# guohaoqiang/Flex

Hardware: AMD Instinct MI355X
Metric: SpMM GFLOPS (2*nnz*k/t) (higher is better)
Workload: dtype f32

## Files before the change

flex_amd/binding.py:

```python
from __future__ import annotations

import ctypes as C
import os
import subprocess

import numpy as np

_HERE = os.path.dirname(os.path.abspath(__file__))
_CSRC = os.path.join(_HERE, "csrc")
_SO = os.path.join(_HERE, "lib", "libflex_spmm.so")

FLEX_ORDER_NATURAL = 0
FLEX_ORDER_RCM = 1
FLEX_ORDER_CLUSTER = 2
FLEX_ORDER_GORDER = 3
FLEX_PLAN_STATS = 0x100
FLEX_PLAN_AUTOTUNE = 0x200
FLEX_PLAN_ROW_RANGE = 0x1000
FLEX_PLAN_XCD_INTERLEAVE = 0x2000
FLEX_PLAN_TRANSPOSE = 0x8000
FLEX_PLAN_MUTABLE_VALUES = 0x10000
FLEX_PLAN_ATTENTION = 0x40000
FLEX_PLAN_ATTENTION_BACKWARD = 0x80000
FLEX_PLAN_BF16 = 0x100000


class FlexError(RuntimeError):
    pass


class _Csr(C.Structure):
    _fields_ = [("m", C.c_int32), ("n", C.c_int32), ("nnz", C.c_int64),
                ("rowPtr", C.c_void_p), ("col", C.c_void_p), ("vals", C.c_void_p)]


class _HostCsr(C.Structure):
    _fields_ = [("m", C.c_int32), ("n", C.c_int32), ("nnz", C.c_int64),
                ("rowPtr", C.POINTER(C.c_uint32)), ("col", C.POINTER(C.c_uint32)),
                ("vals", C.POINTER(C.c_float)),
                ("uni_nb", C.c_int64), ("n_edges_one_way", C.c_int64),
                ("n_edges_asymmetric", C.c_int64),
                ("n_nodes_z_out", C.c_int32), ("n_nodes_z_in", C.c_int32),
                ("n_nodes_z_deg", C.c_int32), ("is_directed", C.c_int32), ("c", C.c_int32)]


class _PlanInfo(C.Structure):
    _fields_ = [("m", C.c_int32), ("n", C.c_int32), ("k", C.c_int32), ("device", C.c_int32),
                ("nnz", C.c_int64), ("n_tasks", C.c_int64), ("n_chunks", C.c_int64),
                ("n_split_rows", C.c_int64), ("n_partials", C.c_int64),
                ("device_bytes", C.c_int64), ("lanes_per_nz", C.c_int32), ("order", C.c_int32),
                ("plan_ms", C.c_double), ("n_slots", C.c_int64), ("two_d", C.c_int32), ("panel_rows", C.c_int32),
                ("n_tiles", C.c_int64), ("tile_nnz", C.c_int64), ("n_records", C.c_int64),
                ("n_blocks", C.c_int64), ("block_rows", C.c_int64), ("block_nnz", C.c_int64), ("block_hot_nnz", C.c_int64),
                ("block_hot_cols", C.c_int64), ("block_panels", C.c_int64), ("block_records", C.c_int64),
                ("n_bundles", C.c_int64), ("bundle_rows", C.c_int64)]


class _PlanStats(C.Structure):
    _fields_ = [("records", C.c_int64), ("cols_wave", C.c_int64), ("cols_wg", C.c_int64),
                ("cols_xcd", C.c_int64), ("reuse_wave", C.c_double), ("reuse_wg", C.c_double),
                ("reuse_xcd", C.c_double), ("gather_bytes", C.c_double), ("l2_bytes", C.c_double),
                ("chunk_rec_max", C.c_int64), ("chunk_rec_mean", C.c_double),
                ("chunk_imb_pct", C.c_double), ("xcd_imb_pct", C.c_double),
                ("split_nnz_pct", C.c_double), ("pad_pct", C.c_double), ("n_workgroups", C.c_int64),
                ("tile_nnz_pct_10", C.c_double), ("tile_nnz_pct_25", C.c_double), ("tile_nnz_pct_50", C.c_double),
                ("tile_mean_fill", C.c_double), ("mfma_tiles", C.c_int64), ("mfma_nnz_pct", C.c_double),
                ("lds_hot_pct_2", C.c_double), ("lds_hot_pct_4", C.c_double), ("lds_u_2", C.c_double), ("lds_u_4", C.c_double)]


class _ClusterTuning(C.Structure):
    _fields_ = [(f, C.c_int32) for f in ("batch", "no_refine", "stretch", "sweeps", "stride")]


class _PlanTuning(C.Structure):
    _fields_ = [(f, C.c_int32) for f in (
        "lanes_per_nz", "chunk_records", "long_row", "piece_records", "row_cost", "xcd_slices", "xcd_balance",
        "chunk_cost", "task_cost", "split_rows", "rec_nt", "unroll", "two_d", "panel_kb", "seg_min", "mfma",
        "mfma_fill_pct", "lds_extra", "host_threads")] + [("cluster", _ClusterTuning)] + [(f, C.c_int32) for f in (
        "blocks", "block_rounds", "block_panel_rows", "block_thr", "block_cap", "block_ablate_retired", "tile_group", "xcd_stretch", "far_first", "bundle", "bundle_len", "rec_pack")] + [("reserved", C.c_int32 * 4)]


TUNING_FIELDS = tuple(f for f, _ in _PlanTuning._fields_ if f not in ("cluster", "block_ablate_retired", "reserved"))
CLUSTER_TUNING_FIELDS = tuple(f for f, _ in _ClusterTuning._fields_)


DEFAULT_TUNING: dict = {}


def _tuning(d) -> "_PlanTuning | None":
    if not d:
        return None
    t = _PlanTuning()
    for key, val in d.items():
        if key in TUNING_FIELDS:
            setattr(t, key, int(val))
        elif key.startswith("cluster_") and key[8:] in CLUSTER_TUNING_FIELDS:
            setattr(t.cluster, key[8:], int(val))
        else:
            raise FlexError(f"unknown tuning knob {key!r} (flex_plan_tuning has: {', '.join(TUNING_FIELDS)}, cluster_*)")
    return t


class _PlanDesc(C.Structure):
    _fields_ = [("struct_size", C.c_size_t), ("A", C.POINTER(_Csr)), ("k", C.c_int), ("ldb", C.c_int), ("ldc", C.c_int),
                ("device", C.c_int), ("flags", C.c_uint), ("row_begin", C.c_int64), ("row_end", C.c_int64),
                ("col_map", C.c_void_p), ("row_map", C.c_void_p), ("tuning", C.POINTER(_PlanTuning))]


class _KernelInfo(C.Structure):
    _fields_ = [("vgprs", C.c_int32), ("sgprs", C.c_int32), ("lds_bytes", C.c_int32), ("scratch_bytes", C.c_int32),
                ("threads_per_block", C.c_int32), ("waves_per_cu", C.c_int32)]


class _Imbalance(C.Structure):
    _fields_ = [("waves", C.c_int64), ("cus_seen", C.c_int32), ("xcds_seen", C.c_int32), ("span_us", C.c_double),
                ("cu_busy_imb_pct", C.c_double), ("cu_end_spread_pct", C.c_double), ("xcd_busy_imb_pct", C.c_double),
                ("xcd_end_spread_pct", C.c_double), ("wave_us_mean", C.c_double), ("wave_us_max", C.c_double)]


class _SoftmaxInfo(C.Structure):
    _fields_ = [(f, C.c_int64) for f in ("rows", "entries", "items", "groups", "rows_empty", "rows_packed", "rows_wave", "rows_block",
                                          "group_entries", "device_bytes")]


class _AttentionInfo(C.Structure):
    _fields_ = [(f, C.c_int64) for f in ("rows", "entries", "items", "groups", "rows_empty", "rows_slot", "rows_wave", "rows_block",
                                          "group_budget", "device_bytes")]


class _AttentionBackwardInfo(C.Structure):
    _fields_ = [(f, C.c_int64) for f in ("columns", "entries", "items", "groups", "columns_empty", "columns_slot", "columns_wave", "columns_block",
                                          "group_budget", "device_bytes")]


class _RecordInfo(C.Structure):
    _fields_ = [("packed", C.c_int32), ("reserved", C.c_int32)] + [(f, C.c_int64) for f in ("records", "wide_records", "exceptions", "stream_bytes")]


class _SynthParams(C.Structure):
    _fields_ = [("n", C.c_int64), ("nnz", C.c_int64), ("alpha", C.c_double),
                ("community", C.c_int64), ("p_in", C.c_double), ("p_near", C.c_double),
                ("near_window", C.c_int32), ("shuffle", C.c_int32), ("gcn_norm", C.c_int32),
                ("directed", C.c_int32), ("seed", C.c_uint64)]


SYMBOLS = [
    "flex_plan_create", "flex_plan_create_ex", "flex_plan_create_ld", "flex_plan_create_mapped", "flex_plan_create_rows", "flex_spmm",
    "flex_plan_destroy", "flex_plan_measure_imbalance", "flex_plan_get_info", "flex_plan_get_stats", "flex_plan_get_tuning", "flex_set_host_threads", "flex_order_cluster_ex", "flex_plan_self_check", "flex_plan_kernel_info", "flex_hbm_probe", "flex_gather_rows", "flex_csv_load", "flex_mtx_load",
    "flex_csv_save", "flex_csr_save_bin", "flex_csr_load_bin", "flex_csr_fingerprint", "flex_perm_save", "flex_perm_load",
    "flex_host_csr_free", "flex_fill_dense_rand", "flex_order_rcm", "flex_order_cluster", "flex_order_gorder", "flex_perm_csr",
    "flex_order_deg", "flex_order_dfs", "flex_order_rabbit", "flex_shard_rows", "flex_synth_graph", "flex_synth_preset", "flex_strerror", "flex_last_hip_error",
    "flex_last_hip_error_string", "flex_abi_version", "flex_plan_set_values", "flex_sddmm",
    "flex_edge_softmax", "flex_edge_softmax_backward", "flex_plan_softmax_info", "flex_attention", "flex_plan_attention_info",
    "flex_attention_backward", "flex_plan_attention_backward_info", "flex_attention_heads", "flex_attention_heads_backward",
    "flex_gat_attention", "flex_gat_attention_backward", "flex_plan_record_info", "flex_plan_read_records",
    "flex_attention_bf16", "flex_attention_bf16_backward", "flex_spmm_bf16", "flex_plan_is_bf16",
    "flex_attention_bias", "flex_attention_bias_backward", "flex_attention_bf16_bias", "flex_attention_bf16_bias_backward",
    "flex_attention_dropout", "flex_attention_dropout_backward", "flex_attention_bf16_dropout", "flex_attention_bf16_dropout_backward",
    "flex_dropout_mask", "flex_gat_attention_dropout", "flex_gat_attention_dropout_backward",
]

_lib = None


def lib_path() -> str:
    return _SO


def build(force: bool = False) -> str:
    if force and os.path.exists(_SO):
        os.remove(_SO)
    subprocess.check_call(["make", "-s", "-C", _CSRC, "all"])
    return _SO


def lib():
    global _lib
    if _lib is None:
        if not os.path.exists(_SO):
            raise FlexError(f"{_SO} is missing: run `python -c 'import __graft_entry__ as g; g.build()'` "
                            "(there is no CPU fallback)")
        try:
            import torch
        except ImportError:
            pass
        L = C.CDLL(_SO)
        vp, i64, i32, u32 = C.c_void_p, C.c_int64, C.c_int, C.c_uint
        L.flex_plan_create.argtypes = [C.POINTER(vp), C.POINTER(_Csr), i32, i32, u32]
        L.flex_plan_create_ex.argtypes = [C.POINTER(vp), C.POINTER(_PlanDesc)]
        L.flex_plan_create_ld.argtypes = [C.POINTER(vp), C.POINTER(_Csr), i32, i32, i32, i32, u32]
        L.flex_plan_create_mapped.argtypes = [C.POINTER(vp), C.POINTER(_Csr), vp, i32, i32, u32]
        L.flex_plan_create_rows.argtypes = [C.POINTER(vp), C.POINTER(_Csr), i64, i64, vp, i32, i32, u32]
        L.flex_spmm.argtypes = [vp, vp, vp, vp]
        L.flex_plan_destroy.argtypes = [vp]
        L.flex_plan_get_info.argtypes = [vp, C.POINTER(_PlanInfo)]
        L.flex_plan_get_stats.argtypes = [vp, C.POINTER(_PlanStats)]
        L.flex_plan_get_tuning.argtypes = [vp, C.POINTER(_PlanTuning)]
        L.flex_set_host_threads.argtypes = [i32]
        L.flex_order_cluster_ex.argtypes = [C.POINTER(_Csr), C.POINTER(_ClusterTuning), vp]
        L.flex_plan_self_check.argtypes = [vp]
        L.flex_plan_measure_imbalance.argtypes = [vp, vp, vp, vp, C.POINTER(_Imbalance)]
        L.flex_plan_kernel_info.argtypes = [vp, C.POINTER(_KernelInfo)]
        L.flex_gather_rows.argtypes = [vp, vp, vp, i64, i32, vp]
        L.flex_hbm_probe.argtypes = [i32, i64, i32, i32, C.POINTER(C.c_double), C.POINTER(C.c_double)]
        L.flex_csv_load.argtypes = [C.c_char_p, C.POINTER(_HostCsr)]
        L.flex_mtx_load.argtypes = [C.c_char_p, i32, C.POINTER(_HostCsr)]
        L.flex_csv_save.argtypes = [C.c_char_p, C.POINTER(_Csr)]
        L.flex_csr_fingerprint.argtypes = [C.POINTER(_Csr)]
        L.flex_csr_fingerprint.restype = C.c_uint64
        L.flex_perm_save.argtypes = [C.c_char_p, vp, i64, C.c_uint64]
        L.flex_perm_load.argtypes = [C.c_char_p, vp, i64, C.c_uint64]
        L.flex_csr_save_bin.argtypes = [C.c_char_p, C.POINTER(_Csr)]
        L.flex_csr_load_bin.argtypes = [C.c_char_p, C.POINTER(_HostCsr)]
        L.flex_host_csr_free.argtypes = [C.POINTER(_HostCsr)]
        L.flex_host_csr_free.restype = None
        L.flex_fill_dense_rand.argtypes = [vp, i64, i32]
        L.flex_order_rcm.argtypes = [C.POINTER(_Csr), vp]
        L.flex_order_cluster.argtypes = [C.POINTER(_Csr), vp]
        L.flex_order_gorder.argtypes = [C.POINTER(_Csr), u32, vp]
        L.flex_order_dfs.argtypes = [C.POINTER(_Csr), vp]
        L.flex_order_rabbit.argtypes = [C.POINTER(_Csr), i32, vp]
        L.flex_order_deg.argtypes = [C.POINTER(_Csr), i32, vp]
        L.flex_synth_preset.argtypes = [C.c_char_p, i32, C.POINTER(_SynthParams)]
        L.flex_perm_csr.argtypes = [C.POINTER(_Csr), vp, vp, vp, vp, vp]
        L.flex_shard_rows.argtypes = [C.POINTER(_Csr), i32, i32, vp]
        L.flex_synth_graph.argtypes = [C.POINTER(_SynthParams), C.POINTER(_HostCsr)]
        L.flex_strerror.argtypes = [i32]
        L.flex_strerror.restype = C.c_char_p
        L.flex_last_hip_error.restype = i32
        L.flex_last_hip_error_string.restype = C.c_char_p
        L.flex_abi_version.restype = i32
        L.flex_plan_softmax_info.argtypes = [vp, C.POINTER(_SoftmaxInfo)]
        L.flex_plan_attention_info.argtypes = [vp, C.POINTER(_AttentionInfo)]
        L.flex_plan_attention_backward_info.argtypes = [vp, C.POINTER(_AttentionBackwardInfo)]
        L.flex_plan_record_info.argtypes = [vp, C.POINTER(_RecordInfo)]
        L.flex_plan_read_records.argtypes = [vp, vp, i64]
        L.flex_plan_is_bf16.argtypes = [vp]
        L.flex_dropout_mask.argtypes = [C.c_uint64, C.c_float, C.c_uint64, C.c_uint64, vp]
        _lib = L
    return _lib


def _values_fn(name: str):
    L = lib()
    f = getattr(L, name)
    if f.argtypes is None:
        vp, fl, i32, u64 = C.c_void_p, C.c_float, C.c_int, C.c_uint64
        f.argtypes = {"flex_plan_set_values": [vp, vp, vp], "flex_sddmm": [vp, vp, vp, vp, vp], "flex_edge_softmax": [vp, vp, fl, vp, vp],
                      "flex_edge_softmax_backward": [vp, vp, vp, fl, vp, vp], "flex_attention": [vp, vp, vp, vp, fl, vp, vp, vp],
                      "flex_attention_backward": [vp, vp, vp, vp, vp, vp, fl, vp, vp, vp, vp, vp],
                      "flex_attention_heads": [vp, i32, vp, vp, vp, fl, vp, vp, vp],
                      "flex_attention_heads_backward": [vp, i32, vp, vp, vp, vp, vp, fl, vp, vp, vp, vp, vp],
                      "flex_attention_bf16": [vp, i32, vp, vp, vp, fl, vp, vp, vp],
                      "flex_attention_bf16_backward": [vp, i32, vp, vp, vp, vp, vp, fl, vp, vp, vp, vp, vp],
                      "flex_attention_bias": [vp, i32, vp, vp, vp, vp, fl, vp, vp, vp],
                      "flex_attention_bias_backward": [vp, i32, vp, vp, vp, vp, vp, fl, vp, vp, vp, vp, vp, vp],
                      "flex_attention_bf16_bias": [vp, i32, vp, vp, vp, vp, fl, vp, vp, vp],
                      "flex_attention_bf16_bias_backward": [vp, i32, vp, vp, vp, vp, vp, fl, vp, vp, vp, vp, vp, vp],
                      "flex_attention_dropout": [vp, i32, vp, vp, vp, vp, fl, fl, u64, vp, vp, vp],
                      "flex_attention_dropout_backward": [vp, i32, vp, vp, vp, vp, vp, fl, fl, u64, vp, vp, vp, vp, vp, vp],
                      "flex_attention_bf16_dropout": [vp, i32, vp, vp, vp, vp, fl, fl, u64, vp, vp, vp],
                      "flex_attention_bf16_dropout_backward": [vp, i32, vp, vp, vp, vp, vp, fl, fl, u64, vp, vp, vp, vp, vp, vp],
                      "flex_spmm_bf16": [vp, vp, vp, vp],
                      "flex_gat_attention": [vp, i32, vp, vp, vp, fl, vp, vp, vp],
                      "flex_gat_attention_backward": [vp, i32, vp, vp, vp, vp, vp, fl, vp, vp, vp, vp, vp],
                      "flex_gat_attention_dropout": [vp, i32, vp, vp, vp, fl, fl, u64, vp, vp, vp],
                      "flex_gat_attention_dropout_backward": [vp, i32, vp, vp, vp, vp, vp, fl, fl, u64, vp, vp, vp, vp, vp]}[name]
    return f


def _check(rc: int, what: str):
    if rc != 0:
        L = lib()
        msg = L.flex_strerror(rc).decode()
        if rc == -3:
            msg += f" [hip {L.flex_last_hip_error()}: {L.flex_last_hip_error_string().decode()}]"
        raise FlexError(f"{what}: {msg} ({rc})")


class HostCsr:

    def __init__(self, rowPtr, col, vals, n=None, **stats):
        self.rowPtr = np.ascontiguousarray(rowPtr, dtype=np.uint32)
        self.col = np.ascontiguousarray(col, dtype=np.uint32)
        self.vals = np.ascontiguousarray(vals, dtype=np.float32)
        self.m = len(self.rowPtr) - 1
        self.n = self.m if n is None else int(n)
        self.nnz = len(self.col)
        self.__dict__.update(stats)

    def view(self) -> _Csr:
        return _Csr(self.m, self.n, self.nnz, self.rowPtr.ctypes.data, self.col.ctypes.data,
                    self.vals.ctypes.data)


def _take(s: _HostCsr) -> HostCsr:
    n = s.n
    try:
        rp = np.ctypeslib.as_array(s.rowPtr, shape=(s.m + 1,)).copy()
        col = np.ctypeslib.as_array(s.col, shape=(max(s.nnz, 1),))[: s.nnz].copy()
        vals = np.ctypeslib.as_array(s.vals, shape=(max(s.nnz, 1),))[: s.nnz].copy()
        stats = {k: getattr(s, k) for k in ("uni_nb", "n_edges_one_way", "n_edges_asymmetric",
                                           "n_nodes_z_out", "n_nodes_z_in", "n_nodes_z_deg",
                                           "is_directed", "c")}
    finally:
        lib().flex_host_csr_free(C.byref(s))
    return HostCsr(rp, col, vals, n=n, **stats)


def csv_load(path: str) -> HostCsr:
    s = _HostCsr()
    _check(lib().flex_csv_load(os.fsencode(path), C.byref(s)), f"flex_csv_load({path})")
    return _take(s)


def mtx_load(path: str, sort_columns: bool = True) -> HostCsr:
    s = _HostCsr()
    _check(lib().flex_mtx_load(os.fsencode(path), int(sort_columns), C.byref(s)), f"flex_mtx_load({path})")
    return _take(s)
# ... 110 lines not shown
def order_gorder(a: HostCsr, window: int = 3) -> np.ndarray:
    rank = np.empty(max(a.m, 1), dtype=np.uint32)
    v = a.view()
    _check(lib().flex_order_gorder(C.byref(v), int(window), rank.ctypes.data), "flex_order_gorder")
    return rank[: a.m]


def order_dfs(a: HostCsr) -> np.ndarray:
    rank = np.empty(max(a.m, 1), dtype=np.uint32)
    v = a.view()
    _check(lib().flex_order_dfs(C.byref(v), rank.ctypes.data), "flex_order_dfs")
    return rank[: a.m]


def order_rabbit(a: HostCsr, is_directed: bool | None = None) -> np.ndarray:
    if is_directed is None:
        is_directed = bool(getattr(a, "is_directed", 0))
    rank = np.empty(max(a.m, 1), dtype=np.uint32)
    v = a.view()
    _check(lib().flex_order_rabbit(C.byref(v), int(bool(is_directed)), rank.ctypes.data), "flex_order_rabbit")
    return rank[: a.m]


def order_deg(a: HostCsr, descending: bool = True) -> np.ndarray:
    rank = np.empty(max(a.m, 1), dtype=np.uint32)
    v = a.view()
    _check(lib().flex_order_deg(C.byref(v), int(descending), rank.ctypes.data), "flex_order_deg")
    return rank[: a.m]


class Plan:

    def __init__(self, a: HostCsr, k: int, device: int = 0, order: int = FLEX_ORDER_NATURAL,
                 vo_mp=None, rows=None, col_map=None, ldb: int | None = None, ldc: int | None = None, tuning: dict | None = None,
                 transpose: bool = False, mutable_values: bool = False, attention: bool = False, attention_backward: bool = False,
                 bf16: bool = False):
        self._h = C.c_void_p()
        self.src_nnz = a.nnz
        if transpose:
            order |= FLEX_PLAN_TRANSPOSE
        if mutable_values:
            order |= FLEX_PLAN_MUTABLE_VALUES
        if attention:
            order |= FLEX_PLAN_ATTENTION
        if attention_backward:
            order |= FLEX_PLAN_ATTENTION_BACKWARD
        if bf16:
            order |= FLEX_PLAN_BF16
        self._keep = (a, vo_mp, col_map)
        v = a.view()
        L = lib()
        tn = _tuning({**DEFAULT_TUNING, **(tuning or {})})
        if tn is not None or ((ldb is not None or ldc is not None) and (rows is not None or vo_mp is not None)):
            cm = None if col_map is None else np.ascontiguousarray(col_map, dtype=np.int32)
            vm = None if vo_mp is None else np.ascontiguousarray(vo_mp, dtype=np.int32)
            self._keep = (a, cm, vm)
            d = _PlanDesc(C.sizeof(_PlanDesc), C.pointer(v), k, ldb or 0, ldc or 0, device,
                          order | (0 if rows is None else FLEX_PLAN_ROW_RANGE),
                          0 if rows is None else int(rows[0]), 0 if rows is None else int(rows[1]),
                          (cm if cm is not None else vm).ctypes.data if (cm is not None or vm is not None) else None,
                          None if vm is None else vm.ctypes.data, None if tn is None else C.pointer(tn))
            rc = L.flex_plan_create_ex(C.byref(self._h), C.byref(d))
        elif rows is not None:
            cm = None if col_map is None else np.ascontiguousarray(col_map, dtype=np.int32)
            self._keep = (a, cm)
            rc = L.flex_plan_create_rows(C.byref(self._h), C.byref(v), int(rows[0]), int(rows[1]),
                                         None if cm is None else cm.ctypes.data, k, device, order)
        elif vo_mp is not None:
            vm = np.ascontiguousarray(vo_mp, dtype=np.int32)
            rc = L.flex_plan_create_mapped(C.byref(self._h), C.byref(v), vm.ctypes.data, k, device, order)
        elif ldb is not None or ldc is not None:
            rc = L.flex_plan_create_ld(C.byref(self._h), C.byref(v), k, ldb or k, ldc or k, device, order)
        else:
            rc = L.flex_plan_create(C.byref(self._h), C.byref(v), k, device, order)
        _check(rc, "flex_plan_create")
        self.k = k
        self._keep = None

    def info(self) -> dict:
        i = _PlanInfo()
        _check(lib().flex_plan_get_info(self._h, C.byref(i)), "flex_plan_get_info")
        d = {f: getattr(i, f) for f, _ in _PlanInfo._fields_}
        d["rec_packed"] = self.record_info()["packed"]
        d["bf16"] = int(lib().flex_plan_is_bf16(self._h))
        return d

    def record_info(self) -> dict:
        ri = _RecordInfo()
        _check(lib().flex_plan_record_info(self._h, C.byref(ri)), "flex_plan_record_info")
        return {f: getattr(ri, f) for f, _ in _RecordInfo._fields_ if f != "reserved"}

    def records(self) -> np.ndarray:
        n = self.record_info()["records"]
        out = np.empty((max(n, 1), 2), dtype=np.uint32)
        _check(lib().flex_plan_read_records(self._h, out.ctypes.data, n), "flex_plan_read_records")
        return out[:n]

    def stats(self) -> dict:
        st = _PlanStats()
        _check(lib().flex_plan_get_stats(self._h, C.byref(st)), "flex_plan_get_stats")
        return {f: getattr(st, f) for f, _ in _PlanStats._fields_}

    def tuning(self) -> dict:
        t = _PlanTuning()
        _check(lib().flex_plan_get_tuning(self._h, C.byref(t)), "flex_plan_get_tuning")
        d = {f: getattr(t, f) for f in TUNING_FIELDS}
        d.update({"cluster_" + f: getattr(t.cluster, f) for f in CLUSTER_TUNING_FIELDS})
        return d

    def kernel_info(self) -> dict:
        ki = _KernelInfo()
        _check(lib().flex_plan_kernel_info(self._h, C.byref(ki)), "flex_plan_kernel_info")
        return {f: getattr(ki, f) for f, _ in _KernelInfo._fields_}

    def measure_imbalance(self, dB_ptr: int, dC_ptr: int, stream: int = 0) -> dict:
        im = _Imbalance()
        _check(lib().flex_plan_measure_imbalance(self._h, dB_ptr, dC_ptr, stream, C.byref(im)), "flex_plan_measure_imbalance")
        return {f: getattr(im, f) for f, _ in _Imbalance._fields_}

    def self_check(self):
        _check(lib().flex_plan_self_check(self._h), "flex_plan_self_check")

    def spmm(self, dB_ptr: int, dC_ptr: int, stream: int = 0):
        _check(lib().flex_spmm(self._h, dB_ptr, dC_ptr, stream), "flex_spmm")

    def spmm_bf16(self, dB_ptr: int, dC_ptr: int, stream: int = 0):
        _check(_values_fn("flex_spmm_bf16")(self._h, dB_ptr, dC_ptr, stream), "flex_spmm_bf16")

    def __call__(self, B, out=None):
        import torch
        i = self.info()
        want = torch.bfloat16 if i["bf16"] else torch.float32
        if B.dtype != want:
            raise TypeError(f"this plan takes {want} operands, got {B.dtype}")
        assert B.is_cuda and B.is_contiguous() and tuple(B.shape) == (i["n"], i["k"])
        if out is None:
            out = torch.empty((i["m"], i["k"]), dtype=want, device=B.device)
        elif out.dtype != want:
            raise TypeError(f"this plan writes {want}, out is {out.dtype}")
        run = self.spmm_bf16 if i["bf16"] else self.spmm
        run(B.data_ptr(), out.data_ptr(), torch.cuda.current_stream(B.device).cuda_stream)
        return out

    def set_values(self, vals, stream: int | None = None):
        import torch
        assert vals.is_cuda and vals.dtype == torch.float32 and vals.is_contiguous() and vals.numel() == self.src_nnz, "float32 cuda [nnz]"
        s = torch.cuda.current_stream(vals.device).cuda_stream if stream is None else stream
        _check(_values_fn("flex_plan_set_values")(self._h, vals.data_ptr(), s), "flex_plan_set_values")

    def sddmm_ptr(self, dG_ptr: int, dB_ptr: int, dOut_ptr: int, stream: int = 0):
        _check(_values_fn("flex_sddmm")(self._h, dG_ptr, dB_ptr, dOut_ptr, stream), "flex_sddmm")

    def sddmm(self, G, B, out=None):
        import torch
        i = self.info()
        assert G.is_cuda and G.dtype == torch.float32 and G.is_contiguous() and tuple(G.shape) == (i["m"], i["k"])
        assert B.is_cuda and B.dtype == torch.float32 and B.is_contiguous() and tuple(B.shape) == (i["n"], i["k"])
        if out is None:
            out = torch.zeros(self.src_nnz, dtype=torch.float32, device=G.device)
        assert out.is_cuda and out.dtype == torch.float32 and out.is_contiguous() and out.numel() == self.src_nnz
        self.sddmm_ptr(G.data_ptr(), B.data_ptr(), out.data_ptr(), torch.cuda.current_stream(G.device).cuda_stream)
        return out

    def softmax_info(self) -> dict:
        i = _SoftmaxInfo()
        _check(lib().flex_plan_softmax_info(self._h, C.byref(i)), "flex_plan_softmax_info")
        return {f: getattr(i, f) for f, _ in _SoftmaxInfo._fields_}

    def edge_softmax_ptr(self, dScores_ptr: int, scale: float, dOut_ptr: int, stream: int = 0):
        _check(_values_fn("flex_edge_softmax")(self._h, dScores_ptr, scale, dOut_ptr, stream), "flex_edge_softmax")

    def edge_softmax_backward_ptr(self, dP_ptr: int, dGradP_ptr: int, scale: float, dGradS_ptr: int, stream: int = 0):
        _check(_values_fn("flex_edge_softmax_backward")(self._h, dP_ptr, dGradP_ptr, scale, dGradS_ptr, stream), "flex_edge_softmax_backward")

    def _edge_vectors(self, *ts):
        import torch
        for t in ts:
            assert t.is_cuda and t.dtype == torch.float32 and t.is_contiguous() and t.numel() == self.src_nnz, "float32 cuda [nnz]"
# ... 403 lines not shown
```

flex_amd/csrc/plan.cpp:

```cpp
#include <algorithm>
#include <atomic>
#include <chrono>
#include <cstddef>
#include <cstdlib>
#include <memory>
#include <new>
#include <vector>

#include "host_parallel.h"
#include "plan.h"

namespace flex {

static thread_local hipError_t g_last_hip = hipSuccess;
void note_hip_error(hipError_t e) { g_last_hip = e; }

int validate_csr(const flex_csr *A) {
    if (!A || A->m < 0 || A->n < 0 || A->nnz < 0) return FLEX_ERR_INVALID;
    if (!A->rowPtr) return FLEX_ERR_INVALID;
    if (A->nnz > 0 && (!A->col || !A->vals)) return FLEX_ERR_INVALID;
    if (A->nnz >= (int64_t(1) << 32)) return FLEX_ERR_UNSUPPORTED;
    if (A->rowPtr[0] != 0 || A->rowPtr[A->m] != static_cast<uint32_t>(A->nnz)) return FLEX_ERR_INVALID;
    for (int32_t r = 0; r < A->m; ++r)
        if (A->rowPtr[r] > A->rowPtr[r + 1]) return FLEX_ERR_INVALID;
// ... 97 lines not shown
    flex_csr csr{};
};

static int transpose_csr(const flex_csr *A, TransposedCsr *t, bool want_entries) {
    int rc = validate_csr(A);
    if (rc) return rc;
    if (A->n >= INT32_MAX) return FLEX_ERR_UNSUPPORTED;
    const size_t nnz = static_cast<size_t>(A->nnz);
    try {
        t->rowPtr.assign(static_cast<size_t>(A->n) + 1, 0u);
        t->col.resize(nnz);
        t->vals.resize(nnz);
        if (want_entries) t->entry.resize(nnz);
    } catch (const std::bad_alloc &) {
        return FLEX_ERR_NOMEM;
    }
    for (size_t e = 0; e < nnz; ++e) ++t->rowPtr[A->col[e] + 1];
    for (int32_t c = 0; c < A->n; ++c) t->rowPtr[c + 1] += t->rowPtr[c];
    std::vector<uint32_t> pos;
    try {
        pos.assign(t->rowPtr.begin(), t->rowPtr.end() - 1);
    } catch (const std::bad_alloc &) {
        return FLEX_ERR_NOMEM;
    }
    for (int32_t r = 0; r < A->m; ++r)
        for (uint32_t e = A->rowPtr[r]; e < A->rowPtr[r + 1]; ++e) {
            const uint32_t d = pos[A->col[e]]++;
            t->col[d] = static_cast<uint32_t>(r);
            t->vals[d] = A->vals[e];
            if (want_entries) t->entry[d] = e;
        }
    t->csr = flex_csr{A->n, A->m, A->nnz, t->rowPtr.data(), nnz ? t->col.data() : nullptr, nnz ? t->vals.data() : nullptr};
    return FLEX_OK;
}

static uint64_t held_entries_fp(const flex_csr *A, bool transposed, int64_t r0, int64_t r1, const int32_t *col_map) {
    auto brow = [&](uint32_t c) { return col_map ? static_cast<uint32_t>(col_map[c]) : c; };
    uint64_t fp = 0;
    if (!transposed) {
        for (uint32_t e = A->rowPtr[r0]; e < A->rowPtr[r1]; ++e) fp += entry_fp(e, brow(A->col[e]));
        return fp;
    }
    for (int32_t r = 0; r < A->m; ++r)
        for (uint32_t e = A->rowPtr[r]; e < A->rowPtr[r + 1]; ++e)
            if (A->col[e] >= r0 && A->col[e] < r1) fp += entry_fp(e, brow(static_cast<uint32_t>(r)));
    return fp;
}

static int create_common(flex_plan **out, const flex_csr *hostA, bool all_rows, int64_t row_begin, int64_t row_end,
                         const int32_t *col_map, const int32_t *dst_map, int k, int device, unsigned flags,
                         int ldb = 0, int ldc = 0, const flex_plan_tuning *tuning_in = nullptr) {
    if (!out) return FLEX_ERR_INVALID;
    *out = nullptr;
    flex_plan_tuning tuning = tuning_in ? *tuning_in : flex_plan_tuning{};
    if (!tuning_ok(tuning)) return FLEX_ERR_INVALID;
    const HostThreadsScope threads_for_this_call(tuning.host_threads);
    if (k <= 0 || device < 0) return FLEX_ERR_INVALID;
    if (ldb == 0) ldb = k;
    if (ldc == 0) ldc = k;
    if (ldb < k || ldc < k) return FLEX_ERR_INVALID;
    const unsigned order = flags & FLEX_ORDER_MASK;
    if (order > FLEX_ORDER_GORDER ||
        (flags & ~(FLEX_ORDER_MASK | FLEX_PLAN_STATS | FLEX_PLAN_AUTOTUNE | FLEX_PLAN_XCD_INTERLEAVE | FLEX_PLAN_TRANSPOSE | FLEX_PLAN_MUTABLE_VALUES | FLEX_PLAN_ATTENTION | FLEX_PLAN_ATTENTION_BACKWARD | FLEX_PLAN_BF16)))
        return FLEX_ERR_INVALID;
    const bool bf16 = (flags & FLEX_PLAN_BF16) != 0;
    if (bf16) {
        if (flags & (FLEX_PLAN_MUTABLE_VALUES | FLEX_PLAN_ATTENTION | FLEX_PLAN_ATTENTION_BACKWARD | FLEX_PLAN_AUTOTUNE)) return FLEX_ERR_UNSUPPORTED;
        if (k % 8 != 0 || ldb % 8 != 0 || ldc % 8 != 0) return FLEX_ERR_UNSUPPORTED;
        if (tuning.mfma == 1 || tuning.blocks == 1 || tuning.split_rows == 1 || tuning.two_d == 1) return FLEX_ERR_UNSUPPORTED;
        tuning.mfma = 2;
        tuning.blocks = 2;
        tuning.split_rows = 2;
        k /= 2;
        ldb /= 2;
        ldc /= 2;
        flags &= ~FLEX_PLAN_BF16;
    }
    const bool mut = (flags & FLEX_PLAN_MUTABLE_VALUES) != 0;
    if (mut) {
        if (tuning.mfma == 1 || tuning.blocks == 1 || tuning.rec_pack == 1) return FLEX_ERR_UNSUPPORTED;
        tuning.mfma = 2;
        tuning.blocks = 2;
        tuning.rec_pack = 2;
    }
    int rc = FLEX_OK;
    const flex_csr *const callerA = hostA;
    const bool transposed = (flags & FLEX_PLAN_TRANSPOSE) != 0;
    const bool attn = (flags & FLEX_PLAN_ATTENTION) != 0;
    if (attn && (transposed || col_map || dst_map || tuning.rec_pack == 1)) return FLEX_ERR_UNSUPPORTED;
    if (attn) tuning.rec_pack = 2;
    const bool attn_bwd = (flags & FLEX_PLAN_ATTENTION_BACKWARD) != 0;
    if (attn_bwd && !attn) return FLEX_ERR_INVALID;
    if (attn_bwd && !all_rows) return FLEX_ERR_UNSUPPORTED;
    flags &= ~(FLEX_PLAN_ATTENTION | FLEX_PLAN_ATTENTION_BACKWARD);
    TransposedCsr at;
    if (transposed) {
        rc = transpose_csr(hostA, &at, mut);
        if (rc) return rc;
        hostA = &at.csr;
        flags &= ~FLEX_PLAN_TRANSPOSE;
    }
    rc = validate_csr(hostA);
    if (rc) return rc;
    if (hostA->m >= INT32_MAX) return FLEX_ERR_UNSUPPORTED;
    if (all_rows) {
        row_begin = 0;
        row_end = hostA->m;
    }
    if (row_begin < 0 || row_end < row_begin || row_end > hostA->m) return FLEX_ERR_INVALID;
    if (col_map)
        for (int32_t c = 0; c < hostA->n; ++c)
            if (col_map[c] < 0 || col_map[c] >= hostA->n) return FLEX_ERR_INVALID;
    if (dst_map)
        for (int64_t r = row_begin; r < row_end; ++r)
            if (dst_map[r] < 0 || dst_map[r] >= hostA->m) return FLEX_ERR_INVALID;
    const auto t0 = std::chrono::steady_clock::now();
    const DeviceScope on(device);
    FLEX_HIP_TRY(on.error());
    std::unique_ptr<flex_plan> p(new (std::nothrow) flex_plan());
    if (!p) return FLEX_ERR_NOMEM;
    p->m = static_cast<int32_t>(row_end - row_begin);
    p->n = hostA->n;
    p->k = k;
    p->ldb = ldb;
    p->ldc = ldc;
    p->bf16 = bf16;
    p->nnz = static_cast<int64_t>(hostA->rowPtr[row_end]) - hostA->rowPtr[row_begin];
    p->device = device;
    std::vector<uint32_t> sched_cache;
    const bool tune = (flags & FLEX_PLAN_AUTOTUNE) != 0;
    const uint32_t *entry_of = transposed && mut && hostA->nnz > 0 ? at.entry.data() : nullptr;
    try {
        rc = build_plan(p.get(), hostA, static_cast<int32_t>(row_begin), static_cast<int32_t>(row_end), col_map, dst_map, flags, tuning,
                        tune ? &sched_cache : nullptr, 0, entry_of);
        if (rc == FLEX_OK && tune) rc = autotune(p, hostA, static_cast<int32_t>(row_begin), static_cast<int32_t>(row_end), col_map, dst_map, flags, tuning, sched_cache, entry_of);
        if (rc == FLEX_OK && mut) {
            p->src_nnz = callerA->nnz;
            p->ent_fp = held_entries_fp(callerA, transposed, row_begin, row_end, col_map);
            if (!transposed) rc = upload_softmax_image(p.get(), callerA->rowPtr, row_begin, row_end);
            else if (all_rows) rc = upload_softmax_image(p.get(), callerA->rowPtr, 0, callerA->m);
        }
        if (rc == FLEX_OK && attn) {
            p->at_ent_fp = held_entries_fp(callerA, false, row_begin, row_end, nullptr);
            if (attn_bwd)
                for (int32_t r = 0; r < callerA->m; ++r)
                    for (uint32_t e = callerA->rowPtr[r]; e < callerA->rowPtr[r + 1]; ++e) p->ab_fp += rowptr_fp(static_cast<uint32_t>(r), e);
            rc = upload_attention_image(p.get(), callerA, row_begin, row_end, attn_bwd);
        }
    } catch (const std::bad_alloc &) {
        rc = FLEX_ERR_NOMEM;
    } catch (...) {
        rc = FLEX_ERR_INVALID;
    }
    if (rc == FLEX_OK && hipDeviceSynchronize() != hipSuccess) rc = FLEX_ERR_HIP;
    if (rc) return rc;
    p->plan_ms = std::chrono::duration<double, std::milli>(std::chrono::steady_clock::now() - t0).count();
    *out = p.release();
    return FLEX_OK;
}

int flex_plan_create(flex_plan **out, const flex_csr *hostA, int k, int device, unsigned flags) {
    if (!hostA) return FLEX_ERR_INVALID;
    return create_common(out, hostA, true, 0, 0, nullptr, nullptr, k, device, flags);
}

int flex_plan_create_ld(flex_plan **out, const flex_csr *hostA, int k, int ldb, int ldc, int device, unsigned flags) {
    if (!hostA || ldb < k || ldc < k) return FLEX_ERR_INVALID;
    return create_common(out, hostA, true, 0, 0, nullptr, nullptr, k, device, flags, ldb, ldc);
}

int flex_plan_create_mapped(flex_plan **out, const flex_csr *hostA, const int32_t *vo_mp, int k, int device,
                            unsigned flags) {
    if (!hostA) return FLEX_ERR_INVALID;
    if (vo_mp && hostA->m != hostA->n) return FLEX_ERR_INVALID;
    return create_common(out, hostA, true, 0, 0, vo_mp, vo_mp, k, device, flags);
}

int flex_plan_create_rows(flex_plan **out, const flex_csr *hostA, int64_t row_begin, int64_t row_end,
                          const int32_t *col_map, int k, int device, unsigned flags) {
    if ((flags & FLEX_ORDER_MASK) != FLEX_ORDER_NATURAL) return FLEX_ERR_INVALID;
    return create_common(out, hostA, false, row_begin, row_end, col_map, nullptr, k, device, flags);
}

int flex_plan_create_ex(flex_plan **out, const flex_plan_desc *d) {
    constexpr size_t kSizeAbi2 = offsetof(flex_plan_desc, tuning);
    if (!d || !d->A || (d->struct_size != sizeof(flex_plan_desc) && d->struct_size != kSizeAbi2)) return FLEX_ERR_INVALID;
    const flex_plan_tuning *tuning = d->struct_size == sizeof(flex_plan_desc) ? d->tuning : nullptr;
    const bool all_rows = (d->flags & FLEX_PLAN_ROW_RANGE) == 0;
    if (all_rows && (d->row_begin != 0 || d->row_end != 0)) return FLEX_ERR_INVALID;
    const int64_t r0 = d->row_begin, r1 = d->row_end;
    if (d->row_map && (!all_rows || d->A->m != d->A->n)) return FLEX_ERR_INVALID;
    if (!all_rows && (d->flags & FLEX_ORDER_MASK) != FLEX_ORDER_NATURAL) return FLEX_ERR_INVALID;
    return create_common(out, d->A, all_rows, r0, r1, d->col_map, d->row_map, d->k, d->device, d->flags & ~FLEX_PLAN_ROW_RANGE, d->ldb, d->ldc, tuning);
}

int flex_spmm(flex_plan *p, const float *dB, float *dC, flex_stream_t stream) {
    if (!p || p->bf16) return FLEX_ERR_INVALID;
    if (p->m == 0) return FLEX_OK;
    if (!dC || (!dB && p->nnz > 0)) return FLEX_ERR_INVALID;
    const DeviceScope on(p->device);
    FLEX_HIP_TRY(on.error());
    const bool vec4 = operands_vec4(p, dB, dC);
    const bool fused = vec4 && p->fused_fixup;
    hipStream_t s = reinterpret_cast<hipStream_t>(stream);
    int rc = FLEX_OK;
    const LaunchGuard guard(p, s);
    if (guard.begin() != FLEX_OK) return FLEX_ERR_INVALID;
    rc = launch_spmm(plan_view(p, fused, nullptr), p->lanes_per_nz, p->off32, vec4, dB, dC, s, p->unroll);
    if (rc == FLEX_OK && !fused) rc = launch_fixup(p->d_partial.get(), p->d_split.get(), p->n_split, p->k, p->ldc, dC, s);
    if (rc == FLEX_OK && p->n_tiles) rc = launch_tiles(tile_view(p), p->off32, dB, dC, p->k, p->ldb, p->ldc, s);
    if (rc == FLEX_OK && p->bk_blocks) rc = launch_blocks(block_view(p), dB, dC, s, vec4);
    if (rc == FLEX_OK) guard.done();
    return rc;
}

int flex_plan_destroy(flex_plan *p) {
    if (!p) return FLEX_OK;
    const DeviceScope on(p->device);
    delete p;
    return FLEX_OK;
}

int flex_plan_get_info(const flex_plan *p, flex_plan_info *o) {
    if (!p || !o) return FLEX_ERR_INVALID;
    o->m = p->m;
    o->n = p->n;
    o->k = p->k * p->elems_per_word();
    o->device = p->device;
    o->nnz = p->nnz;
    o->n_tasks = p->n_tasks;
    o->n_chunks = p->n_chunks;
    o->n_split_rows = p->n_split;
    o->n_partials = p->n_partials;
    o->device_bytes = p->device_bytes;
    o->lanes_per_nz = p->lanes_per_nz;
    o->order = static_cast<int32_t>(p->order);
    o->plan_ms = p->plan_ms;
    o->n_slots = p->n_slots;
    o->two_d = p->two_d ? 1 : 0;
    o->n_tiles = p->n_tiles;
    o->tile_nnz = p->tile_nnz;
    o->n_records = p->n_records;
    o->panel_rows = p->two_d ? static_cast<int32_t>(p->panel_rows) : 0;
    o->n_blocks = p->bk_blocks;
    o->block_rows = p->bk_rows;
    o->block_nnz = p->bk_nnz;
    o->block_hot_nnz = p->bk_hot_nnz;
    o->block_hot_cols = p->bk_hot_cols;
    o->block_panels = p->bk_panels;
    o->block_records = static_cast<int64_t>(p->d_bk_rec.size());
    o->n_bundles = p->n_bundles;
    o->bundle_rows = p->bundle_rows;
    return FLEX_OK;
}

int flex_plan_record_info(const flex_plan *p, flex_record_info *o) {
    if (!p || !o) return FLEX_ERR_INVALID;
    const int64_t exceptions = static_cast<int64_t>(p->d_exc.size());
    const int64_t bytes = p->rec_packed ? 6 * (p->n_records - p->wide_records) + 8 * (p->wide_records + exceptions) : 8 * p->n_records;
    *o = flex_record_info{p->rec_packed ? 1 : 0, 0, p->n_records, p->wide_records, exceptions, bytes};
    return FLEX_OK;
}

int flex_plan_softmax_info(const flex_plan *p, flex_softmax_info *o) {
    if (!p || !o || !p->mutable_vals) return FLEX_ERR_INVALID;
    if (!p->sm_ok) return FLEX_ERR_UNSUPPORTED;
    *o = flex_softmax_info{p->sm_rows, p->sm_entries, static_cast<int64_t>(p->d_sm_item.size()), p->n_sm_groups, p->sm_class_rows[3],
                           p->sm_class_rows[kSmPacked], p->sm_class_rows[kSmWaveRow], p->sm_class_rows[kSmBlockRow], p->sm_group_budget, p->sm_bytes};
    return FLEX_OK;
}

int flex_plan_attention_backward_info(const flex_plan *p, flex_attention_backward_info *o) {
    if (!p || !o || !p->ab_ok) return FLEX_ERR_INVALID;
    *o = flex_attention_backward_info{p->ab_cols, p->at_entries, static_cast<int64_t>(p->d_ab_item.size()), p->n_ab_groups, p->ab_class_cols[3],
                                      p->ab_class_cols[kAtSlot], p->ab_class_cols[kAtWave], p->ab_class_cols[kAtBlock], p->ab_group_budget, p->ab_bytes};
    return FLEX_OK;
}

int flex_plan_attention_info(const flex_plan *p, flex_attention_info *o) {
    if (!p || !o || !p->at_ok) return FLEX_ERR_INVALID;
    *o = flex_attention_info{p->at_rows, p->at_entries, static_cast<int64_t>(p->d_at_item.size()), p->n_at_groups, p->at_class_rows[3],
                             p->at_class_rows[kAtSlot], p->at_class_rows[kAtWave], p->at_class_rows[kAtBlock], p->at_group_budget, p->at_bytes};
    return FLEX_OK;
}

// ... 68 lines not shown
```

flex_amd/csrc/plan.h:

```cpp
#pragma once
#include <algorithm>
#include <cstdlib>
#include <memory>
#include <new>
#include <type_traits>
#include <utility>
#include <vector>

#include "internal.h"

namespace flex {

template <class T>
class DeviceArray {
  public:
    DeviceArray() = default;
    DeviceArray(DeviceArray &&o) noexcept : ptr_(std::exchange(o.ptr_, nullptr)), n_(std::exchange(o.n_, 0)) {}
    DeviceArray &operator=(DeviceArray o) noexcept {
        std::swap(ptr_, o.ptr_);
        std::swap(n_, o.n_);
        return *this;
    }
    ~DeviceArray() { if (ptr_) (void)hipFree(ptr_); }
    T *get() const { return ptr_; }
    size_t size() const { return n_; }
    hipError_t allocate(size_t n) {
        *this = DeviceArray();
        const hipError_t e = hipMalloc(reinterpret_cast<void **>(&ptr_), std::max<size_t>(n, 1) * sizeof(T));
        if (e != hipSuccess) ptr_ = nullptr;
        else n_ = n;
        return e;
    }
    template <class A>
    int upload(const std::vector<T, A> &h, int64_t *device_bytes) {
        FLEX_HIP_TRY(allocate(h.size()));
        if (!h.empty()) FLEX_HIP_TRY(hipMemcpy(ptr_, h.data(), h.size() * sizeof(T), hipMemcpyHostToDevice));
        *device_bytes += static_cast<int64_t>(std::max<size_t>(h.size(), 1) * sizeof(T));
        return FLEX_OK;
    }

  private:
    T *ptr_ = nullptr;
    size_t n_ = 0;
};

class DeviceScope {
  public:
    explicit DeviceScope(int dev) {
        err_ = hipGetDevice(&prev_);
        if (err_ == hipSuccess && prev_ != dev) {
            err_ = hipSetDevice(dev);
            switched_ = err_ == hipSuccess;
        }
    }
    ~DeviceScope() { if (switched_) (void)hipSetDevice(prev_); }
    DeviceScope(const DeviceScope &) = delete;
    DeviceScope &operator=(const DeviceScope &) = delete;
    hipError_t error() const { return err_; }

  private:
    int prev_ = -1;
    bool switched_ = false;
    hipError_t err_ = hipSuccess;
};

}

struct flex_plan {
    int32_t m = 0, n = 0, k = 0, device = 0;
    int32_t ldb = 0, ldc = 0;
    bool bf16 = false;
    int elems_per_word() const { return bf16 ? 2 : 1; }
    int64_t nnz = 0;
    int lanes_per_nz = 0;
    bool off32 = false;
    bool xcd_remap = true;
    unsigned lds_extra = 0;
    bool rec_nt = false;
    uint32_t tile_group = 0;
    int unroll = 0;
    unsigned order = 0;
    flex::DeviceArray<uint2> d_rec;
    flex::DeviceArray<uint32_t> d_t_beg, d_t_dst;
    flex::DeviceArray<uint2> d_t_aux;
    flex::DeviceArray<uint4> d_chunk;
    flex::DeviceArray<uint32_t> d_bd_rows;
    flex::DeviceArray<uint2> d_chunk_bd;
    bool rec_packed = false;
    flex::DeviceArray<float> d_rec_val;
    flex::DeviceArray<uint16_t> d_rec_dcol;
    flex::DeviceArray<uint32_t> d_t_col0;
    flex::DeviceArray<uint2> d_chunk_exc, d_exc;
    int64_t n_records = 0;
    int64_t wide_records = 0;
    uint64_t rec_fp = 0;
    uint32_t n_bundles = 0;
    int64_t bundle_rows = 0;
    flex::DeviceArray<float> d_partial;
    flex::DeviceArray<flex::SplitRow> d_split;
    flex::DeviceArray<uint32_t> d_split_cnt;
    bool fused_fixup = false;
    bool two_d = false;
    flex::DeviceArray<float> d_tile_a;
    flex::DeviceArray<uint32_t> d_tile_boff, d_tile_mask, d_rt_ptr, d_rt_rows;
    uint32_t n_tiles = 0, n_row_tiles = 0;
    int64_t tile_nnz = 0;
    int64_t tile_hist[3] = {0, 0, 0}, tile_cells = 0;
    bool tile_hist_valid = false;
    uint32_t panel_rows = 0;
    flex::DeviceArray<uint4> d_bk_hdr;
    flex::DeviceArray<uint2> d_bk_wstart, d_bk_rec;
    flex::DeviceArray<uint32_t> d_bk_cnt, d_bk_hcol, d_bk_brow, d_bk_link;
    uint32_t bk_blocks = 0, bk_rounds = 0, bk_panel_rows = 0;
    int64_t bk_rows = 0, bk_nnz = 0, bk_hot_nnz = 0, bk_hot_cols = 0, bk_panels = 0;
    uint32_t n_tasks = 0, n_chunks = 0, n_slots = 0, n_split = 0, n_partials = 0;
    int64_t c_rows = 0;
    int64_t device_bytes = 0;
    double plan_ms = 0;
    double lds_hot[2] = {0, 0}, lds_u[2] = {0, 0};
    bool has_stats = false;
    flex_plan_stats stats{};
    flex_plan_tuning tuning{};
    hipStream_t last_stream = nullptr;
    bool launched = false;
    bool mutable_vals = false;
    flex::DeviceArray<uint32_t> d_src;
    flex::DeviceArray<float> d_vrec;
    flex::DeviceArray<uint4> d_seg;
    flex::DeviceArray<uint4> d_sd_item;
    flex::DeviceArray<uint32_t> d_sd_grp;
    uint32_t n_sd_groups = 0;
    int64_t src_nnz = 0;
    uint64_t ent_fp = 0;
    bool sm_ok = false;
    flex::DeviceArray<uint32_t> d_sm_rowptr;
    flex::DeviceArray<uint4> d_sm_item;
    flex::DeviceArray<uint32_t> d_sm_grp;
    uint32_t n_sm_groups = 0, n_sm_wave_items = 0, n_sm_block_rows = 0, sm_group_budget = 0;
    int64_t sm_rows = 0, sm_entries = 0, sm_bytes = 0;
    int64_t sm_class_rows[4] = {0, 0, 0, 0};
    uint64_t sm_fp = 0;
    bool at_ok = false;
    flex::DeviceArray<uint32_t> d_at_rowptr;
    flex::DeviceArray<uint32_t> d_at_src;
    flex::DeviceArray<uint4> d_at_item;
    flex::DeviceArray<uint32_t> d_at_grp;
    uint32_t n_at_groups = 0, n_at_wave_items = 0, n_at_block_rows = 0, at_group_budget = 0, at_first_entry = 0;
    int64_t at_rows = 0, at_entries = 0, at_bytes = 0;
    int64_t at_class_rows[4] = {0, 0, 0, 0};
    uint64_t at_fp = 0, at_ent_fp = 0;
    bool ab_ok = false;
    flex::DeviceArray<uint32_t> d_ab_colptr;
    flex::DeviceArray<uint2> d_ab_ent;
    flex::DeviceArray<uint4> d_ab_item;
    flex::DeviceArray<uint32_t> d_ab_grp;
    uint32_t n_ab_groups = 0, n_ab_wave_items = 0, n_ab_block_cols = 0, ab_group_budget = 0;
    int64_t ab_cols = 0, ab_bytes = 0;
    int64_t ab_class_cols[4] = {0, 0, 0, 0};
    uint64_t ab_fp = 0;
};

namespace flex {


template <typename T>
struct default_init_allocator : std::allocator<T> {
    template <typename U>
    struct rebind {
        using other = default_init_allocator<U>;
    };
    template <typename U>
    void construct(U *ptr) noexcept(std::is_nothrow_default_constructible_v<U>) {
        ::new (static_cast<void *>(ptr)) U;
    }
    template <typename U, typename... Args>
    void construct(U *ptr, Args &&...args) {
        ::new (static_cast<void *>(ptr)) U(std::forward<Args>(args)...);
    }
};
using RecordVec = std::vector<uint2, default_init_allocator<uint2>>;

inline PlanView plan_view(const flex_plan *p, bool fused, uint64_t *trace) {
    return PlanView{p->d_rec.get(), p->d_t_beg.get(), p->d_t_dst.get(), p->d_t_aux.get(), p->d_chunk.get(), p->d_partial.get(), p->d_split.get(),
                    p->d_split_cnt.get(), fused ? 1u : 0u, p->n_slots, p->k, p->ldb, p->ldc,
                    p->xcd_remap ? 1u : 0u, p->lds_extra, p->rec_nt ? 1u : 0u, p->tile_group, trace, p->d_bd_rows.get(), p->d_chunk_bd.get(),
// ... 99 lines not shown
```

flex_amd/csrc/plan_build.cpp:

```cpp
#include <algorithm>
#include <atomic>
#include <chrono>
#include <cstdio>
#include <cmath>
#include <cstring>
#include <new>
#include <numeric>

#include "host_parallel.h"
#include "plan.h"

namespace flex {

namespace {

struct Piece {
    uint32_t spos;
    uint32_t beg, end;
    uint32_t phase;
    uint32_t own_chunk;
};
constexpr uint32_t kFarPhase = 0xFFFFFFFEu;
struct TaskSpec {
    uint32_t ref;
    uint32_t rows;
    uint32_t steps;
};
constexpr uint32_t kMaxTasksPerWave = 63;

class PlanBuilder {
   public:
    PlanBuilder(flex_plan *plan, const flex_csr *csr, int32_t row_begin, int32_t row_end, const int32_t *col_map_, const int32_t *dst_map_,
                unsigned flags_, const flex_plan_tuning &tuning, std::vector<uint32_t> *sched_cache_, int force_G_, bool want_blocks_ = false,
                const uint32_t *entry_of_ = nullptr)
        : p(plan), A(csr), r0(row_begin), r1(row_end), m(row_end - row_begin), k(plan->k), col_map(col_map_), dst_map(dst_map_),
          flags(flags_), order(flags_ & FLEX_ORDER_MASK), force_G(force_G_), want_blocks(want_blocks_), mut((flags_ & FLEX_PLAN_MUTABLE_VALUES) != 0),
          entry_of(entry_of_), tn(tuning), sched(sched_cache_ ? *sched_cache_ : sched_local),
          have_cache(sched_cache_ != nullptr), timing(plan_timing_enabled()), t_last(std::chrono::steady_clock::now()) {}

    int schedule_only(std::vector<uint32_t> **sched_out, std::vector<uint32_t> **colpos_out) {
        if (order > FLEX_ORDER_GORDER) return FLEX_ERR_INVALID;
        if (order != FLEX_ORDER_NATURAL && (A->m != A->n || r0 != 0 || r1 != A->m)) return FLEX_ERR_INVALID;
        choose_tile_width();
        const int rc = order_rows();
        lap("row schedule");
        *sched_out = &sched;
        *colpos_out = &colpos;
        return rc;
    }

    int run() {
        if (order > FLEX_ORDER_GORDER) return FLEX_ERR_INVALID;
        if (order != FLEX_ORDER_NATURAL && (A->m != A->n || r0 != 0 || r1 != A->m)) return FLEX_ERR_INVALID;
        p->order = order;
        int rc;
        choose_tile_width();
        if ((rc = order_rows())) return rc;
        lap("row schedule");
        if ((flags & FLEX_PLAN_STATS) && m > 0) {
            p->lds_hot[0] = 100.0 * estimate_hot_share(A, sched, 480, 2, 4, &p->lds_u[0]);
            p->lds_hot[1] = 100.0 * estimate_hot_share(A, sched, 480, 4, 4, &p->lds_u[1]);
        }
        if ((rc = route_dense_tiles())) return rc;
        lap("dense-tile detector");
        if (want_blocks && tiles.nnz == 0 && m > 0) {
            if ((rc = route_hot_blocks())) return rc;
            lap("hot blocks");
        }
        if (mut && (tiles.nnz || p->bk_blocks)) return FLEX_ERR_UNSUPPORTED;
        read_knobs();
        if ((rc = cut_rows_into_pieces())) return rc;
        lap("pieces");
        slice_rows_for_xcds();
        order_pieces();
        lap("emission order");
        number_split_rows();
        form_tasks();
        if ((rc = pack_tasks_into_chunks())) return rc;
        fill_records();
        lap("records and tasks");
        pack_records();
        lap("record packing");
        if ((rc = upload_tasks())) return rc;
        lap("upload records/tasks");
        if ((rc = build_chunk_table())) return rc;
        lap("chunk table, stats");
        if (mut) {
            if ((rc = upload_value_image())) return rc;
            lap("value image");
        }
        return FLEX_OK;
    }

   private:
    flex_plan *const p;
    const flex_csr *A;
    const int32_t r0, r1, m;
    const int k;
    const int32_t *const col_map;
    const int32_t *const dst_map;
    const unsigned flags, order;
    const int force_G;
    const bool want_blocks;
    const bool mut;
    const uint32_t *const entry_of;
    const flex_plan_tuning &tn;
    std::vector<uint32_t> sched_local;
    std::vector<uint32_t> &sched;
    const bool have_cache;
    const bool timing;
    std::chrono::steady_clock::time_point t_last;

    int G = 8;
    uint32_t S = 8;
    double avg_deg = 0.0;
    std::vector<uint32_t> colpos;
    DenseTiles tiles;
    flex_csr A_f{};
    std::vector<uint32_t> f_rowptr, f_col;
    std::vector<float> f_vals;
    uint32_t wave_nnz = 0, row_cost = 16, long_row = 0, piece_len = 0, seg_min = 4, pshift = 0, far_window = 0;
    bool two_d = false;
    bool xcd_dealt = false;
    std::vector<Piece> pieces;
    std::vector<uint32_t> row_first_piece;
    std::vector<uint32_t> pcol;
    std::vector<float> pval;
    std::vector<uint32_t> pent;
    const uint32_t *rcol = nullptr;
    const float *rval = nullptr;
    uint32_t slice_row[kXcds + 1] = {0};
    std::vector<uint32_t> emit;
    bool bundles_on = false;
    uint32_t bundle_len = 0;
    std::vector<TaskSpec> tasks;
    std::vector<uint32_t> bundle_piece;
    std::vector<uint32_t> bd_rows;
    std::vector<uint2> chunk_bd;
    uint32_t n_bundles = 0;
    int64_t bundle_rows = 0;
    std::vector<SplitRow> split;
    std::vector<uint32_t> row_sidx, row_first_partial;
    uint32_t n_partials = 0;
    int64_t split_nnz = 0;
    std::vector<uint32_t> t_beg, t_dst, w_task;
    std::vector<uint2> t_aux;
    RecordVec rec;
    std::vector<uint32_t> rsrc;
    std::vector<float> rvals;
    uint32_t slice_chunk[kXcds + 1] = {0};
    size_t n_records = 0;
    int pack_mode = 0;
    bool packed = false;
    std::vector<float, default_init_allocator<float>> pk_val;
    std::vector<uint16_t, default_init_allocator<uint16_t>> pk_dcol;
    std::vector<uint32_t> pk_col0;
    std::vector<uint2> pk_exc, pk_chunk_exc;
    RecordVec pk_wide;
    int64_t pk_wide_records = 0;

    void lap(const char *what) {
        if (!timing) return;
        const auto now = std::chrono::steady_clock::now();
        std::fprintf(stderr, "plan: %-22s %8.1f ms\n", what, std::chrono::duration<double, std::milli>(now - t_last).count());
        t_last = now;
    }
    static long pick(int32_t given, long rule) { return given > 0 ? given : rule; }
    uint32_t dst_of(uint32_t r) const { return dst_map ? static_cast<uint32_t>(dst_map[r]) : r - static_cast<uint32_t>(r0); }
    int64_t slice_nnz() const { return static_cast<int64_t>(A->rowPtr[r1]) - A->rowPtr[r0]; }

    void choose_tile_width() {
        avg_deg = m > 0 ? static_cast<double>(A->rowPtr[r1] - A->rowPtr[r0]) / m : 0.0;
        G = 8;
        while (4 * G < k && G < 64) G <<= 1;
        const bool narrow_ok = k <= 16 && k % 4 == 0;
        if (force_G) {
            G = std::min(G, force_G);
        } else if (const int g_t = tn.lanes_per_nz; g_t == 8 || g_t == 16 || g_t == 32 || g_t == 64 || (g_t == 4 && narrow_ok)) {
            G = g_t == 4 ? 4 : std::min<int>(G, g_t);
        } else if (narrow_ok && (avg_deg >= 8.0 || tn.bundle == 1 || (tn.bundle != 2 && bundle_rule()))) {
            G = 4;
        } else {
            G = std::min(G, 32);
            if (avg_deg >= 24.0) G = std::min(G, 16);
            if (avg_deg >= 128.0) G = std::min(G, 8);
            if (tn.bundle == 1 || (tn.bundle != 2 && bundle_rule())) G = std::min(G, 16);
        }
        S = 64u / static_cast<uint32_t>(G);
        p->lanes_per_nz = G;
        p->off32 = static_cast<uint64_t>(A->n) * static_cast<uint64_t>(p->ldb) * 4u <= (uint64_t(1) << 32);
    }

    int order_rows() {
        if (have_cache && sched.size() == static_cast<size_t>(m) && m > 0) {
        } else if (sched.assign(static_cast<size_t>(m), 0u); order != FLEX_ORDER_NATURAL) {
            std::vector<uint32_t> rank;
            const int rc = order == FLEX_ORDER_RCM       ? order_rcm_host(m, A->rowPtr, A->col, rank)
                           : order == FLEX_ORDER_CLUSTER ? order_cluster_host(m, A->rowPtr, A->col, rank, &tn.cluster)
                                                         : order_gorder_host(m, A->rowPtr, A->col, 3, rank);
            if (rc) {
                sched.clear();
                return rc;
            }
            for (int32_t r = 0; r < m; ++r) sched[rank[r]] = static_cast<uint32_t>(r);
        } else {
// ... 70 lines not shown
    int route_hot_blocks() {
        BlockKnobs kn;
        const int32_t rd = tn.block_rounds;
        if (rd == 2 || rd == 4 || rd == 8) kn.rounds = static_cast<uint32_t>(rd);
        else if (rd != 0) return FLEX_ERR_INVALID;
        else if (m < 8 * 256 * 480) kn.rounds = m < 8 * 256 * 240 ? 2 : 4;
        if (tn.block_panel_rows) {
            if (tn.block_panel_rows % 4 != 0 || tn.block_panel_rows > static_cast<int32_t>(kBkPanelMax)) return FLEX_ERR_INVALID;
            kn.panel_rows = static_cast<uint32_t>(tn.block_panel_rows);
        }
        kn.thr = tn.block_thr ? static_cast<uint32_t>(tn.block_thr) : 3u;
        kn.cap = tn.block_cap ? static_cast<uint32_t>(std::min<int32_t>(tn.block_cap, 60000)) : static_cast<uint32_t>(std::clamp(1.5 * avg_deg, 32.0, 4096.0));
        kn.min_last_panel = std::min<uint32_t>(32, kn.panel_rows / 4);
        BlockImage img;
        std::vector<uint8_t> hot_mask;
        const uint32_t row_bytes32 = static_cast<uint32_t>(p->ldb) * 4u;
        int rc;
        if ((rc = build_blocks(A, sched, colpos, col_map, dst_map, r0, row_bytes32, kn, img, hot_mask))) return rc;
        flex_plan_tuning &u = p->tuning;
        u.blocks = 1;
        u.block_rounds = static_cast<int32_t>(kn.rounds);
        u.block_panel_rows = static_cast<int32_t>(kn.panel_rows);
        u.block_thr = static_cast<int32_t>(kn.thr);
        u.block_cap = static_cast<int32_t>(kn.cap);
        if (timing)
            std::fprintf(stderr, "plan: hot blocks %u x %u slots, %lld rows, %lld nnz; candidates %.1f %%, hot %.1f %% (left cold: panel budget %.1f %%, short last panel %.1f %%, runs beyond %u steps %.1f %%), "
                         "u %.2f, records / hot %.2f, panels / block %.1f\n", img.n_blocks, kn.rounds * kBkRowsPerRound, static_cast<long long>(img.rows), static_cast<long long>(img.nnz),
                         100.0 * img.cand_nnz / std::max<int64_t>(img.nnz, 1), 100.0 * img.hot_nnz / std::max<int64_t>(img.nnz, 1), 100.0 * img.lost_panels / std::max<int64_t>(img.nnz, 1),
                         100.0 * img.lost_last / std::max<int64_t>(img.nnz, 1), kn.run_max, 100.0 * img.lost_run / std::max<int64_t>(img.nnz, 1),
                         static_cast<double>(img.hot_nnz) / std::max<int64_t>(img.hot_cols, 1), static_cast<double>(img.rec.size()) / std::max<int64_t>(img.hot_nnz, 1),
                         static_cast<double>(img.panels) / std::max<uint32_t>(img.n_blocks, 1));
        if (img.hot_nnz == 0) return FLEX_OK;
        if ((rc = p->d_bk_hdr.upload(img.hdr, &p->device_bytes))) return rc;
        if ((rc = p->d_bk_wstart.upload(img.wstart, &p->device_bytes))) return rc;
        if ((rc = p->d_bk_cnt.upload(img.cnt, &p->device_bytes))) return rc;
        if ((rc = p->d_bk_hcol.upload(img.hcol, &p->device_bytes))) return rc;
        if ((rc = p->d_bk_brow.upload(img.brow, &p->device_bytes))) return rc;
        if ((rc = p->d_bk_link.upload(img.link, &p->device_bytes))) return rc;
        if ((rc = p->d_bk_rec.upload(img.rec, &p->device_bytes))) return rc;
        p->bk_blocks = img.n_blocks;
        p->bk_rounds = img.rounds;
        p->bk_panel_rows = img.panel_rows;
        p->bk_rows = img.rows;
        p->bk_nnz = img.nnz;
        p->bk_hot_nnz = img.hot_nnz;
        p->bk_hot_cols = img.hot_cols;
        p->bk_panels = img.panels;
        img = BlockImage{};
        keep_unmarked(hot_mask);
        choose_tile_width();
        return FLEX_OK;
    }

    void read_knobs() {
        const long lo_budget = G <= 8 ? 128 : 96;
        long auto_budget = std::clamp<long>(static_cast<long>((G <= 8 ? 16.0 : 8.0) * avg_deg), lo_budget, G <= 8 ? 512 : 256);
        const bool bundles_expected = tn.two_d != 1 && S >= kBundleMinSlots && m > 0 && (tn.bundle == 1 || (tn.bundle != 2 && bundle_rule()));
        const long n_rec = static_cast<long>(A->rowPtr[r1] - A->rowPtr[r0]);
        auto_budget = std::min(auto_budget, std::max<long>(G <= 8 || bundles_expected ? 64 : lo_budget, n_rec / 2048));
        wave_nnz = static_cast<uint32_t>(pick(tn.chunk_records, auto_budget));
        row_cost = static_cast<uint32_t>(pick(tn.row_cost, 16));
        const long remap_env = tn.xcd_slices;
        const bool interleave = order == FLEX_ORDER_RCM || order == FLEX_ORDER_GORDER || (flags & FLEX_PLAN_XCD_INTERLEAVE) != 0;
        p->xcd_remap = remap_env == 1 || remap_env == 3 || (remap_env != 2 && !interleave);
        xcd_dealt = remap_env == 3;
        p->lds_extra = static_cast<unsigned>(std::max(0, tn.lds_extra)) & ~15u;
        const long nt_env = tn.rec_nt;
        const int ktiles = (k + 4 * G - 1) / (4 * G);
        const uint64_t stream_bytes = static_cast<uint64_t>(A->rowPtr[r1] - A->rowPtr[r0]) * 8u;
        p->tile_group = (ktiles >= 2 && tn.tile_group > 1) ? static_cast<uint32_t>(tn.tile_group) : 0u;
        p->rec_nt = nt_env == 1 || (nt_env != 2 && p->tile_group == 0 && stream_bytes >= (ktiles >= 2 ? (32ull << 20) : (1ull << 30)));
        p->unroll = tn.unroll == 8 ? 8 : 0;
        long whole_row = wave_nnz;
        if (n_rec / std::max<long>(wave_nnz, 1) <= 4096) whole_row = std::max<long>(wave_nnz, std::min<long>(4L * wave_nnz, 12L * S * (G >= 32 ? 8 : 4)));
        long_row = static_cast<uint32_t>(pick(tn.long_row, whole_row));
        piece_len = std::max<uint32_t>(S, static_cast<uint32_t>(pick(tn.piece_records, wave_nnz)) / S * S);

        two_d = tn.two_d == 1 && m > 0;
        const uint64_t tile_bytes = 16ull * static_cast<uint64_t>(G);
        const uint64_t panel_bytes = static_cast<uint64_t>(pick(tn.panel_kb, 2048)) << 10;
        pshift = 0;
        while ((2ull << pshift) * tile_bytes <= panel_bytes) ++pshift;
        seg_min = static_cast<uint32_t>(pick(tn.seg_min, 4));
        bundles_on = bundles_expected && !two_d;
        bundle_len = static_cast<uint32_t>(pick(tn.bundle_len, S >= 8 ? 12 : 16));
        const bool pack_shape = !two_d && !mut && k % 4 == 0 && p->ldb % 4 == 0 && p->ldc % 4 == 0;
        pack_mode = !pack_shape || tn.rec_pack == 2 ? 0 : tn.rec_pack == 1 ? 2 : (ktiles >= 2 && stream_bytes >= (32ull << 20)) ? 1 : 0;
        far_window = two_d ? 0u : static_cast<uint32_t>(std::max(0, tn.far_first));
        p->tuning.far_first = static_cast<int32_t>(far_window);
        flex_plan_tuning &u = p->tuning;
        u.lanes_per_nz = G;
        u.chunk_records = static_cast<int32_t>(wave_nnz);
        u.long_row = static_cast<int32_t>(long_row);
        u.piece_records = static_cast<int32_t>(piece_len);
        u.row_cost = static_cast<int32_t>(row_cost);
        u.xcd_slices = xcd_dealt ? 3 : p->xcd_remap ? 1 : 2;
        u.rec_nt = p->rec_nt ? 1 : 2;
        u.tile_group = p->tile_group ? static_cast<int32_t>(p->tile_group) : 1;
        u.unroll = p->unroll;
        u.two_d = two_d ? 1 : 0;
        u.panel_kb = static_cast<int32_t>(panel_bytes >> 10);
        u.seg_min = static_cast<int32_t>(seg_min);
        u.lds_extra = static_cast<int32_t>(p->lds_extra);
        u.host_threads = host_threads();
        u.cluster = tn.cluster;
    }

    bool fills_the_chip() const {
        const double budget = std::clamp(16.0 * avg_deg, 128.0, 512.0);
        return (static_cast<double>(slice_nnz()) + 16.0 * m) / budget >= 8192.0;
    }
    bool bundle_rule() const { return fills_the_chip() || avg_deg < 16.0; }

    void cut_run(std::vector<Piece> &out, uint32_t spos, uint32_t b, uint32_t e, uint32_t phase) const {
        const uint32_t len = e - b;
        if (len <= long_row) {
            out.push_back({spos, b, e, phase, 0u});
            return;
        }
        constexpr uint32_t kMaxPieces = 256;
        const uint32_t nchunk = std::min<uint32_t>((len + piece_len - 1) / piece_len, kMaxPieces);
        const uint32_t per = ((len + nchunk - 1) / nchunk + S - 1) / S * S;
        for (uint32_t c0 = b; c0 < e; c0 += per) out.push_back({spos, c0, std::min(e, c0 + per), phase, 1u});
    }

    int cut_rows_into_pieces() {
        row_first_piece.assign(static_cast<size_t>(m) + 1, 0u);
        rcol = A->col;
        rval = A->vals;
        if (two_d) return cut_by_column_panel();
        pieces.reserve(static_cast<size_t>(m) + 1024);
        for (int32_t i = 0; i < m; ++i) {
            const uint32_t r = sched[i];
            row_first_piece[i] = static_cast<uint32_t>(pieces.size());
            cut_run(pieces, static_cast<uint32_t>(i), A->rowPtr[r], A->rowPtr[r + 1], 0u);
        }
        row_first_piece[m] = static_cast<uint32_t>(pieces.size());
        return FLEX_OK;
    }

    int cut_by_column_panel() {
        const uint32_t e_base = A->rowPtr[r0];
        pcol.resize(static_cast<size_t>(slice_nnz()));
        pval.resize(static_cast<size_t>(slice_nnz()));
        if (mut) pent.resize(static_cast<size_t>(slice_nnz()));
        constexpr int64_t kBlk = 1024;
        const int64_t nblk = (m + kBlk - 1) / kBlk;
        std::vector<std::vector<Piece>> blk(static_cast<size_t>(nblk));
        std::vector<uint32_t> row_np(static_cast<size_t>(m), 0u);
        std::atomic<int> failed{0};
        parallel_chunks(nblk, [&](int64_t b) {
            try {
                std::vector<Piece> &out = blk[static_cast<size_t>(b)];
                std::vector<uint64_t> key;
                std::vector<uint32_t> run_beg, run_pan;
                for (int64_t i = b * kBlk; i < std::min<int64_t>(m, (b + 1) * kBlk); ++i) {
                    const uint32_t r = sched[i];
                    const uint32_t e0 = A->rowPtr[r], e1 = A->rowPtr[r + 1], len = e1 - e0;
                    const size_t before = out.size();
                    const uint32_t o0 = e0 - e_base;
                    if (len == 0) {
                        out.push_back({static_cast<uint32_t>(i), o0, o0, kFarPhase, 0u});
                        row_np[i] = 1;
                        continue;
                    }
                    key.resize(len);
                    bool sorted = true;
                    for (uint32_t z = 0; z < len; ++z) {
                        const uint32_t c = A->col[e0 + z];
                        const uint32_t pan = (colpos.empty() ? c : colpos[c]) >> pshift;
                        key[z] = (static_cast<uint64_t>(pan) << 32) | z;
                        sorted = sorted && (z == 0 || key[z - 1] <= key[z]);
                    }
                    if (!sorted) std::sort(key.begin(), key.end());
                    run_beg.clear();
                    run_pan.clear();
                    for (uint32_t z = 0; z < len; ++z)
                        if (z == 0 || (key[z] >> 32) != (key[z - 1] >> 32)) {
                            run_beg.push_back(z);
                            run_pan.push_back(static_cast<uint32_t>(key[z] >> 32));
                        }
                    run_beg.push_back(len);
                    uint32_t o = o0, n_far = 0, n_kept = 0;
                    auto copy_run = [&](size_t q) {
                        for (uint32_t z = run_beg[q]; z < run_beg[q + 1]; ++z) {
                            const uint32_t e = e0 + static_cast<uint32_t>(key[z] & 0xFFFFFFFFu);
                            pcol[o] = A->col[e];
                            pval[o] = A->vals[e];
                            if (mut) pent[o] = e;
                            ++o;
                        }
                    };
                    for (size_t q = 0; q + 1 < run_beg.size(); ++q) {
                        const uint32_t cnt = run_beg[q + 1] - run_beg[q];
                        if (cnt < seg_min) {
                            n_far += cnt;
                            continue;
                        }
                        copy_run(q);
                        ++n_kept;
                        cut_run(out, static_cast<uint32_t>(i), o - cnt, o, run_pan[q] + 1);
                    }
                    const uint32_t far_beg = o;
                    if (n_far) {
                        for (size_t q = 0; q + 1 < run_beg.size(); ++q)
                            if (run_beg[q + 1] - run_beg[q] < seg_min) copy_run(q);
                        if (n_far < seg_min && n_kept > 0 && out.back().own_chunk == 0) out.back().end = o;
                        else cut_run(out, static_cast<uint32_t>(i), far_beg, o, kFarPhase);
                    }
                    row_np[i] = static_cast<uint32_t>(out.size() - before);
                }
            } catch (...) {
                failed.store(1);
            }
        });
        if (failed.load()) return FLEX_ERR_NOMEM;
        size_t total = 0;
        for (int32_t i = 0; i < m; ++i) {
            row_first_piece[i] = static_cast<uint32_t>(total);
            total += row_np[i];
        }
        row_first_piece[m] = static_cast<uint32_t>(total);
        if (total >= (size_t(1) << 31)) return FLEX_ERR_UNSUPPORTED;
        pieces.resize(total);
        parallel_chunks(nblk, [&](int64_t b) {
            const std::vector<Piece> &src = blk[static_cast<size_t>(b)];
            if (!src.empty()) std::copy(src.begin(), src.end(), pieces.begin() + row_first_piece[b * kBlk]);
        });
        rcol = pcol.data();
        rval = pval.data();
        return FLEX_OK;
    }

    void slice_rows_for_xcds() {
        std::fill(slice_row, slice_row + kXcds, 0u);
        slice_row[kXcds] = static_cast<uint32_t>(m);
        if (!two_d) return;
        std::vector<uint64_t> cum(static_cast<size_t>(m) + 1, 0);
        for (int32_t i = 0; i < m; ++i) {
            const uint32_t r = sched[i];
            cum[i + 1] = cum[i] + (A->rowPtr[r + 1] - A->rowPtr[r]) + row_cost;
        }
        for (int x = 1; x < kXcds; ++x)
            slice_row[x] = std::max<uint32_t>(slice_row[x - 1], static_cast<uint32_t>(std::lower_bound(cum.begin(), cum.end(), cum[m] * x / kXcds) - cum.begin()));
    }

    void order_pieces() {
        emit.resize(pieces.size());
        std::iota(emit.begin(), emit.end(), 0u);
        if (!two_d) return;
        parallel_chunks(kXcds, [&](int64_t x) {
            auto b = emit.begin() + row_first_piece[slice_row[x]], e = emit.begin() + row_first_piece[slice_row[x + 1]];
            std::stable_sort(b, e, [&](uint32_t u, uint32_t v) { return pieces[u].phase < pieces[v].phase; });
        });
    }

    void number_split_rows() {
        row_sidx.assign(static_cast<size_t>(m), 0u);
        row_first_partial.assign(static_cast<size_t>(m), 0u);
        for (int32_t i = 0; i < m; ++i) {
            const uint32_t np = row_first_piece[i + 1] - row_first_piece[i];
            if (np <= 1) continue;
            const uint32_t r = sched[i];
            row_sidx[i] = static_cast<uint32_t>(split.size());
            row_first_partial[i] = n_partials;
            split.push_back({dst_of(r), n_partials, np});
            n_partials += np;
            split_nnz += A->rowPtr[r + 1] - A->rowPtr[r];
        }
    }

    void form_tasks() {
        const uint32_t n_pieces = static_cast<uint32_t>(pieces.size());
        tasks.clear();
        tasks.reserve(n_pieces);
        if (n_partials >= kBundleFlag) bundles_on = false;
        p->tuning.bundle = bundles_on ? 1 : 2;
        p->tuning.bundle_len = bundles_on ? static_cast<int32_t>(bundle_len) : 0;
        if (!bundles_on) {
            for (uint32_t t = 0; t < n_pieces; ++t) tasks.push_back({t, 0u, 0u});
            return;
        }
        constexpr uint32_t kRowEnd2 = 5, kBundleEnd2 = 3;
        auto len_of = [&](uint32_t e) { return pieces[emit[e]].end - pieces[emit[e]].beg; };
        std::vector<uint32_t> buf;
        auto flush_buf = [&]() {
            std::stable_sort(buf.begin(), buf.end(), [&](uint32_t a, uint32_t b) { return len_of(a) > len_of(b); });
            for (size_t g = 0; g < buf.size(); g += S) {
                const uint32_t n = static_cast<uint32_t>(std::min<size_t>(S, buf.size() - g));
                const uint32_t steps = len_of(buf[g]);
                uint32_t alone2 = 0;
                for (uint32_t s = 0; s < n; ++s) alone2 += 2 * ((len_of(buf[g + s]) + S - 1) / S) + kRowEnd2;
                if (n >= 2 && 2 * steps + kBundleEnd2 <= alone2) {
                    tasks.push_back({static_cast<uint32_t>(bundle_piece.size()), n, steps});
                    for (uint32_t s = 0; s < n; ++s) bundle_piece.push_back(buf[g + s]);
                    ++n_bundles;
                    bundle_rows += n;
                } else {
                    for (uint32_t s = 0; s < n; ++s) tasks.push_back({buf[g + s], 0u, 0u});
                }
            }
            buf.clear();
        };
        for (uint32_t e = 0; e < n_pieces; ++e) {
            const Piece &pc = pieces[emit[e]];
            if (pc.own_chunk == 0 && pc.end - pc.beg <= bundle_len) {
                buf.push_back(e);
                if (buf.size() == 8u * S) flush_buf();
            } else {
                tasks.push_back({e, 0u, 0u});
            }
        }
        flush_buf();
    }

    int pack_tasks_into_chunks() {
        const uint32_t n_tasks = static_cast<uint32_t>(tasks.size());
        t_beg.resize(static_cast<size_t>(n_tasks) + 1);
        t_dst.resize(n_tasks);
        t_aux.resize(n_tasks);
        uint64_t pos = 0;
        uint32_t wave_cost = 0, cur_phase = 0, prev_own = 0, bd_first = 0;
        int cur_slice = 0;
        for (uint32_t t = 0; t < n_tasks; ++t) {
            const TaskSpec &ts = tasks[t];
            const Piece &pc = pieces[emit[ts.rows ? bundle_piece[ts.ref] : ts.ref]];
            const uint32_t own = ts.rows ? 0u : pc.own_chunk;
            const uint32_t len = ts.rows ? ts.steps * S : pc.end - pc.beg;
            bool fresh = w_task.empty() || wave_cost >= wave_nnz || t - w_task.back() >= kMaxTasksPerWave || own || prev_own;
            if (ts.rows && static_cast<uint32_t>(bd_rows.size()) - bd_first + S > kBundleRowsPerChunk) fresh = true;
            if (two_d) {
                while (pc.spos >= slice_row[cur_slice + 1]) {
                    slice_chunk[++cur_slice] = static_cast<uint32_t>(w_task.size());
                    fresh = true;
                }
                if (pc.phase != cur_phase) fresh = true;
                cur_phase = pc.phase;
            }
            if (fresh) {
                if (!w_task.empty()) chunk_bd.push_back(make_uint2(bd_first, static_cast<uint32_t>(bd_rows.size()) - bd_first));
                bd_first = static_cast<uint32_t>(bd_rows.size());
                w_task.push_back(t);
                wave_cost = 0;
            }
            wave_cost += len + row_cost;
            prev_own = own;
            t_beg[t] = static_cast<uint32_t>(pos);
            if (ts.rows) {
                t_dst[t] = kPartialFlag | kBundleFlag | (static_cast<uint32_t>(bd_rows.size()) - bd_first);
                t_aux[t] = make_uint2(static_cast<uint32_t>(bd_rows.size()), ts.steps);
                for (uint32_t s = 0; s < S; ++s) {
                    if (s < ts.rows) {
                        const Piece &row = pieces[emit[bundle_piece[ts.ref + s]]];
                        bd_rows.push_back(dst_of(sched[row.spos]) | (row.end == row.beg ? kBundleZero : 0u));
                    } else {
                        bd_rows.push_back(kBundleNoRow);
                    }
                }
                pos += len;
            } else {
                pos += (len + S - 1) / S * S;
            }
            if (pos >= (uint64_t(1) << 32)) return FLEX_ERR_UNSUPPORTED;
        }
        t_beg[n_tasks] = static_cast<uint32_t>(pos);
        if (!w_task.empty()) chunk_bd.push_back(make_uint2(bd_first, static_cast<uint32_t>(bd_rows.size()) - bd_first));
        w_task.push_back(n_tasks);
        if (m == 0) w_task.assign(1, 0u);
        if (two_d)
            while (cur_slice < kXcds) slice_chunk[++cur_slice] = static_cast<uint32_t>(w_task.size() - 1);
        rec.resize(static_cast<size_t>(pos));
        return FLEX_OK;
    }

    void fill_records() {
        const uint32_t n_tasks = static_cast<uint32_t>(tasks.size());
        const uint32_t row_bytes32 = static_cast<uint32_t>(p->ldb) * 4u;
        constexpr int64_t kTaskBlk = 4096;
        auto record_of = [&](uint32_t e) {
            uint32_t c = rcol[e];
            if (col_map) c = static_cast<uint32_t>(col_map[c]);
            uint32_t bits;
            std::memcpy(&bits, &rval[e], 4);
            return make_uint2(p->off32 ? c * row_bytes32 : c, bits);
        };
        if (mut) {
            rsrc.assign(rec.size(), kNoEntry);
            rvals.assign(rec.size(), 0.0f);
        }
        auto note_entry = [&](size_t at, uint32_t e) {
            if (!mut) return;
            const uint32_t i = two_d ? pent[e] : e;
            rsrc[at] = entry_of ? entry_of[i] : i;
            rvals[at] = rval[e];
        };
        parallel_chunks((static_cast<int64_t>(n_tasks) + kTaskBlk - 1) / kTaskBlk, [&](int64_t b) {
            for (int64_t t = b * kTaskBlk; t < std::min<int64_t>(n_tasks, (b + 1) * kTaskBlk); ++t) {
                const TaskSpec &ts = tasks[t];
                uint2 *const base = rec.data() + t_beg[t];
                if (ts.rows) {
                    for (uint32_t s = 0; s < S; ++s) {
                        uint32_t len = 0;
                        if (s < ts.rows) {
                            const Piece &pc = pieces[emit[bundle_piece[ts.ref + s]]];
                            len = pc.end - pc.beg;
                            for (uint32_t j = 0; j < len; ++j) {
                                base[static_cast<size_t>(j) * S + s] = record_of(pc.beg + j);
                                note_entry(t_beg[t] + static_cast<size_t>(j) * S + s, pc.beg + j);
                            }
                        }
                        if (len > 0) pad_values(base + s, len, ts.steps - len, S);
                        else
                            for (uint32_t j = 0; j < ts.steps; ++j) base[static_cast<size_t>(j) * S + s] = make_uint2(base[static_cast<size_t>(j) * S].x, 0u);
                    }
                    continue;
                }
                const uint32_t pi = emit[ts.ref];
                const Piece &pc = pieces[pi];
                const uint32_t i = pc.spos, r = sched[i];
                const uint32_t np = row_first_piece[i + 1] - row_first_piece[i];
                if (np > 1) {
                    t_dst[t] = kPartialFlag | (row_first_partial[i] + (pi - row_first_piece[i]));
                    t_aux[t] = make_uint2(row_sidx[i], np);
                } else {
                    t_dst[t] = dst_of(r);
                    t_aux[t] = make_uint2(0u, 0u);
                }
                uint2 *o = base;
                if (far_window == 0) {
                    for (uint32_t e = pc.beg; e < pc.end; ++e) {
                        note_entry(static_cast<size_t>(o - rec.data()), e);
                        *o++ = record_of(e);
                    }
                } else {
                    const auto is_far = [&](uint32_t e) {
                        const uint32_t c = rcol[e];
                        const int64_t cp = colpos.empty() ? static_cast<int64_t>(c) : static_cast<int64_t>(colpos[c]);
                        const int64_t d = cp - static_cast<int64_t>(colpos.empty() ? r : i);
                        return (d < 0 ? -d : d) > static_cast<int64_t>(far_window);
                    };
                    for (int near = 0; near < 2; ++near)
                        for (uint32_t e = pc.beg; e < pc.end; ++e)
                            if (is_far(e) != (near == 1)) {
                                note_entry(static_cast<size_t>(o - rec.data()), e);
                                *o++ = record_of(e);
                            }
                }
                uint2 *const end = rec.data() + t_beg[t + 1];
                if (o > base) pad_values(base, static_cast<uint32_t>(o - base), static_cast<uint32_t>(end - o), 1u);
            }
        });
        pcol = std::vector<uint32_t>();
// ... 119 lines not shown
            if ((rc = p->d_rt_ptr.upload(tiles.rt_ptr, &p->device_bytes))) return rc;
            if ((rc = p->d_rt_rows.upload(tiles.rt_rows, &p->device_bytes))) return rc;
        }
        return FLEX_OK;
    }

    int upload_value_image() {
        std::vector<uint4> seg, item;
        std::vector<uint32_t> grp;
        const uint32_t W = static_cast<uint32_t>(sddmm_lanes(k)), per_pass = 4u * (64u / W);
        uint32_t g_cost = 0, g_items = 0;
        auto add_run = [&](uint32_t first, uint32_t len, uint32_t n_pad, uint32_t stride, uint32_t row) {
            if (len > 0 && n_pad > 0) seg.push_back(make_uint4(first, len, n_pad, stride));
            for (uint32_t j = 0; j < len; j += kSdItemRecords) {
                const uint32_t cnt = std::min(kSdItemRecords, len - j), cost = (cnt + per_pass - 1) / per_pass + 1;
                if (grp.empty() || g_cost + cost > kSdGroupCost || g_items == kSdGroupItems) {
                    grp.push_back(static_cast<uint32_t>(item.size()));
                    g_cost = g_items = 0;
                }
                item.push_back(make_uint4(first + j * stride, cnt, stride, row));
                g_cost += cost;
                ++g_items;
            }
        };
        for (size_t t = 0; t < tasks.size(); ++t) {
            const TaskSpec &ts = tasks[t];
            if (ts.rows) {
                for (uint32_t s = 0; s < ts.rows; ++s) {
                    const Piece &pc = pieces[emit[bundle_piece[ts.ref + s]]];
                    const uint32_t len = pc.end - pc.beg;
                    add_run(t_beg[t] + s, len, ts.steps - len, S, dst_of(sched[pc.spos]));
                }
            } else {
                const Piece &pc = pieces[emit[ts.ref]];
                const uint32_t len = pc.end - pc.beg;
                add_run(t_beg[t], len, t_beg[t + 1] - t_beg[t] - len, 1u, dst_of(sched[pc.spos]));
            }
        }
        grp.push_back(static_cast<uint32_t>(item.size()));
        p->mutable_vals = true;
        p->tuning.blocks = 2;
        p->n_sd_groups = static_cast<uint32_t>(grp.size() - 1);
        int rc;
        if ((rc = p->d_src.upload(rsrc, &p->device_bytes))) return rc;
        if ((rc = p->d_vrec.upload(rvals, &p->device_bytes))) return rc;
        if ((rc = p->d_seg.upload(seg, &p->device_bytes))) return rc;
        if ((rc = p->d_sd_item.upload(item, &p->device_bytes))) return rc;
        if ((rc = p->d_sd_grp.upload(grp, &p->device_bytes))) return rc;
        rsrc = std::vector<uint32_t>();
        rvals = std::vector<float>();
        return FLEX_OK;
    }

    int build_chunk_table() {
        const uint32_t n_real = static_cast<uint32_t>(w_task.size() - 1);
        auto header = [&](uint32_t c) {
            return make_uint4(w_task[c], w_task[c + 1] - w_task[c], t_beg[w_task[c]], t_beg[w_task[c + 1]]);
        };
        std::vector<uint4> chunk;
        std::vector<uint2> cbd;
        std::vector<uint2> cex;
        auto place = [&](size_t at, uint32_t c) {
            chunk[at] = header(c);
            if (n_bundles) cbd[at] = chunk_bd[c];
            if (packed) cex[at] = pk_chunk_exc[c];
        };
        p->tuning.xcd_balance = tn.xcd_balance == 2 ? 2 : 1;
        if (xcd_dealt && !two_d && n_real >= 8u * kXcds * kWavesPerBlock) {
            const uint32_t per = static_cast<uint32_t>(pick(tn.xcd_stretch, 256)) * kWavesPerBlock;
            p->tuning.xcd_stretch = static_cast<int32_t>(per / kWavesPerBlock);
            const uint32_t n_st = (n_real + per - 1) / per;
            uint32_t len[kXcds] = {};
            for (uint32_t s = 0; s < n_st; ++s) len[s % kXcds] += std::min(per, n_real - s * per);
            uint32_t longest = *std::max_element(len, len + kXcds);
            longest = (longest + kWavesPerBlock - 1) / kWavesPerBlock * kWavesPerBlock;
            chunk.assign(static_cast<size_t>(longest) * kXcds, make_uint4(0u, 0u, 0u, 0u));
            if (n_bundles) cbd.assign(chunk.size(), make_uint2(0u, 0u));
            if (packed) cex.assign(chunk.size(), make_uint2(0u, 0u));
            uint32_t at[kXcds] = {};
            for (uint32_t s = 0; s < n_st; ++s) {
                const uint32_t x = s % kXcds, c0 = s * per, c1 = std::min(n_real, c0 + per);
                for (uint32_t c = c0; c < c1; ++c) place(static_cast<size_t>(x) * longest + at[x]++, c);
            }
        } else if (two_d || (p->xcd_remap && n_real >= 8u * kXcds * kWavesPerBlock && tn.xcd_balance != 2)) {
            uint32_t cut[kXcds + 1];
            cut[0] = 0;
            cut[kXcds] = n_real;
            if (two_d) {
                for (uint32_t x = 1; x < kXcds; ++x) cut[x] = slice_chunk[x];
            } else {
                const uint64_t chunk_cost = static_cast<uint64_t>(pick(tn.chunk_cost, 16)) * 32u;
                const uint64_t task_cost = static_cast<uint64_t>(pick(tn.task_cost, 2)) * 32u;
                p->tuning.chunk_cost = static_cast<int32_t>(chunk_cost / 32u);
                p->tuning.task_cost = static_cast<int32_t>(task_cost / 32u);
                std::vector<uint64_t> cum(n_real + 1, 0);
                for (uint32_t c = 0; c < n_real; ++c) {
                    const uint4 h = header(c);
                    cum[c + 1] = cum[c] + static_cast<uint64_t>(h.w - h.z) * static_cast<uint32_t>(G) + task_cost * h.y + chunk_cost;
                }
                for (uint32_t x = 1; x < kXcds; ++x) {
                    const uint64_t want = cum[n_real] * x / kXcds;
                    uint32_t c = static_cast<uint32_t>(std::lower_bound(cum.begin(), cum.end(), want) - cum.begin());
                    c = (c + kWavesPerBlock / 2) / kWavesPerBlock * kWavesPerBlock;
                    cut[x] = std::clamp(c, cut[x - 1], n_real);
                }
            }
            uint32_t longest = 0;
            for (uint32_t x = 0; x < kXcds; ++x) longest = std::max(longest, cut[x + 1] - cut[x]);
            longest = (longest + kWavesPerBlock - 1) / kWavesPerBlock * kWavesPerBlock;
            chunk.assign(static_cast<size_t>(longest) * kXcds, make_uint4(0u, 0u, 0u, 0u));
            if (n_bundles) cbd.assign(chunk.size(), make_uint2(0u, 0u));
            if (packed) cex.assign(chunk.size(), make_uint2(0u, 0u));
            for (uint32_t x = 0; x < kXcds; ++x)
                for (uint32_t c = cut[x]; c < cut[x + 1]; ++c) place(static_cast<size_t>(x) * longest + (c - cut[x]), c);
        } else {
            chunk.resize(n_real);
            if (n_bundles) cbd.resize(n_real);
            if (packed) cex.resize(n_real);
            for (uint32_t c = 0; c < n_real; ++c) place(c, c);
        }
        p->n_chunks = n_real;
        p->n_slots = static_cast<uint32_t>(chunk.size());
        int rc;
        if ((rc = p->d_chunk.upload(chunk, &p->device_bytes))) return rc;
        if (n_bundles && (rc = p->d_chunk_bd.upload(cbd, &p->device_bytes))) return rc;
        if (packed && (rc = p->d_chunk_exc.upload(cex, &p->device_bytes))) return rc;
        if (flags & FLEX_PLAN_STATS) collect_stats(p, rec, chunk, split_nnz);
        if ((rc = p->d_split.upload(split, &p->device_bytes))) return rc;
        const size_t ktiles = (static_cast<size_t>(k) + 4 * G - 1) / (4 * G);
        std::vector<uint32_t> zeros(std::max<size_t>(1, split.size() * ktiles), 0u);
        if ((rc = p->d_split_cnt.upload(zeros, &p->device_bytes))) return rc;
        const size_t n_pfloats = std::max<size_t>(1, static_cast<size_t>(n_partials) * k * p->elems_per_word());
        const double madds = static_cast<double>(slice_nnz()) * k * p->elems_per_word();
        p->fused_fixup = tn.split_rows == 1 || (tn.split_rows != 2 && madds <= 4e8);
        p->tuning.split_rows = p->fused_fixup ? 1 : 2;
        FLEX_HIP_TRY(p->d_partial.allocate(n_pfloats));
        p->device_bytes += static_cast<int64_t>(n_pfloats * sizeof(float));
        return FLEX_OK;
    }
};

}

int build_plan(flex_plan *p, const flex_csr *A, int32_t r0, int32_t r1, const int32_t *col_map, const int32_t *dst_map, unsigned flags,
               const flex_plan_tuning &tuning, std::vector<uint32_t> *sched_cache, int force_G, const uint32_t *entry_of) try {
    const bool block_shapes = p->k % 4 == 0 && p->k >= 64 && p->ldb % 4 == 0 && p->ldc % 4 == 0 &&
                              static_cast<uint64_t>(A->n) * static_cast<uint64_t>(p->ldb) * 4u <= (uint64_t(1) << 32);
    const bool can_block = block_shapes && force_G == 0 && r1 > r0 && tuning.mfma != 1 && tuning.two_d != 1 && tuning.blocks != 2;
    bool want_blocks = tuning.blocks == 1 && can_block;
    std::vector<uint32_t> local_cache;
    const int64_t nnz_in = static_cast<int64_t>(A->rowPtr[r1]) - A->rowPtr[r0];
    if (tuning.blocks == 0 && can_block && static_cast<int64_t>(r1 - r0) >= 480 * 2048 && nnz_in >= 48ll * (r1 - r0)) {
        if (!sched_cache) sched_cache = &local_cache;
        std::vector<uint32_t> *sched = nullptr, *colpos = nullptr;
        int rc;
        {
            PlanBuilder pre(p, A, r0, r1, col_map, dst_map, flags, tuning, sched_cache, 0);
            if ((rc = pre.schedule_only(&sched, &colpos))) return rc;
        }
        const double share = estimate_hot_share(A, *sched_cache, 480, 3, 16);
        if (plan_timing_enabled()) std::fprintf(stderr, "plan: hot share of 480-row blocks (thr 3, every 16th) %.3f\n", share);
        want_blocks = share >= 0.72;
    }
    return PlanBuilder(p, A, r0, r1, col_map, dst_map, flags, tuning, sched_cache, force_G, want_blocks, entry_of).run();
} catch (const std::bad_alloc &) {
    return FLEX_ERR_NOMEM;
}

int upload_softmax_image(flex_plan *p, const uint32_t *rowPtr, int64_t r0, int64_t r1) try {
    const size_t rows = static_cast<size_t>(r1 - r0);
    std::vector<uint32_t> rp(rowPtr + r0, rowPtr + r1 + 1), grp;
// ... 170 lines not shown
```

flex_amd/csrc/plan_check.cpp:

```cpp
#include <algorithm>
#include <new>

#include "plan.h"

using namespace flex;

namespace flex {

void collect_stats(flex_plan *p, const RecordVec &rec, const std::vector<uint4> &chunk, int64_t split_nnz) {
    flex_plan_stats &st = p->stats;
    st = flex_plan_stats{};
    const uint32_t n_chunks = static_cast<uint32_t>(chunk.size());
    uint32_t nblk = (n_chunks + kWavesPerBlock - 1) / kWavesPerBlock;
    nblk = (nblk + kXcds - 1) / kXcds * kXcds;
    const uint32_t cpx = std::max(1u, nblk / kXcds);
    const uint32_t row_bytes32 = static_cast<uint32_t>(p->ldb) * 4u;
    std::vector<uint32_t> seen_wave(p->n, 0u), seen_wg(p->n, 0u), seen_xcd(p->n, 0u);
    int64_t xcd_rec[kXcds] = {0};
    for (uint32_t c = 0; c < n_chunks; ++c) {
        const uint32_t wg = c / kWavesPerBlock;
        const uint32_t xcd = p->xcd_remap ? std::min<uint32_t>(wg / cpx, kXcds - 1) : wg % kXcds;
        const uint32_t n_rec = chunk[c].w - chunk[c].z;
        if (chunk[c].y == 0) continue;
        for (uint32_t z = chunk[c].z; z < chunk[c].w; ++z) {
// ... 44 lines not shown
    if (!p->rec_packed) {
        if (p->d_rec.size() != n_rec) return FLEX_ERR_FORMAT;
        return read_back(p->d_rec, rec) ? FLEX_OK : FLEX_ERR_HIP;
    }
    if (p->d_rec_val.size() != n_rec || p->d_rec_dcol.size() != n_rec || p->d_t_col0.size() != p->n_tasks || p->d_chunk_exc.size() != chunk.size() ||
        p->d_rec.size() != static_cast<size_t>(p->wide_records) || (p->wide_records == 0) != (p->d_rec.get() == nullptr))
        return FLEX_ERR_FORMAT;
    std::vector<float> val;
    std::vector<uint16_t> dcol;
    std::vector<uint32_t> col0;
    std::vector<uint2> cex, exc, wide;
    if (!read_back(p->d_rec_val, val) || !read_back(p->d_rec_dcol, dcol) || !read_back(p->d_t_col0, col0) || !read_back(p->d_chunk_exc, cex) ||
        !read_back(p->d_exc, exc) || !read_back(p->d_rec, wide))
        return FLEX_ERR_HIP;
    const uint32_t row_bytes32 = static_cast<uint32_t>(p->ldb) * 4u;
    rec.assign(n_rec, make_uint2(0u, 0u));
    uint64_t exc_used = 0, wide_used = 0;
    for (size_t ci = 0; ci < chunk.size(); ++ci) {
        const uint4 &c = chunk[ci];
        const uint2 ce = cex[ci];
        if (c.y == 0) {
            if (ce.x | ce.y) return FLEX_ERR_FORMAT;
            continue;
        }
        if (static_cast<uint64_t>(c.x) + c.y > p->n_tasks || c.z != t_beg[c.x] || c.w != t_beg[c.x + c.y] || c.z > c.w || c.w > n_rec) return FLEX_ERR_FORMAT;
        if (ce.y & kChunkWide) {
            if (ce.y != kChunkWide || ce.x != wide_used || wide_used + (c.w - c.z) > wide.size()) return FLEX_ERR_FORMAT;
            std::copy(wide.begin() + static_cast<ptrdiff_t>(wide_used), wide.begin() + static_cast<ptrdiff_t>(wide_used + (c.w - c.z)), rec.begin() + c.z);
            wide_used += c.w - c.z;
            continue;
        }
        if (ce.x != exc_used || exc_used + ce.y > exc.size()) return FLEX_ERR_FORMAT;
        const uint2 *e = exc.data() + exc_used, *const e_end = e + ce.y;
        for (uint32_t t = c.x; t < c.x + c.y; ++t) {
            if (t_beg[t] > t_beg[t + 1] || t_beg[t + 1] > c.w) return FLEX_ERR_FORMAT;
            uint32_t col = col0[t];
            for (uint32_t i = t_beg[t]; i < t_beg[t + 1]; ++i) {
                uint32_t d = dcol[i];
                if (e < e_end && e->x == i - c.z) {
                    if (i == t_beg[t] || (e->y & 0xFFFFu) != 0 || e->y == 0) return FLEX_ERR_FORMAT;
                    d |= e->y;
                    ++e;
                }
                if (i == t_beg[t] && d != 0) return FLEX_ERR_FORMAT;
                col += d;
                if (col >= static_cast<uint64_t>(p->n)) return FLEX_ERR_FORMAT;
                rec[i] = make_uint2(p->off32 ? col * row_bytes32 : col, __builtin_bit_cast(uint32_t, val[i]));
            }
        }
        if (e != e_end) return FLEX_ERR_FORMAT;
        exc_used += ce.y;
    }
    if (exc_used != exc.size() || wide_used != wide.size()) return FLEX_ERR_FORMAT;
    uint64_t fp = 0;
    for (size_t i = 0; i < n_rec; ++i) fp += record_fp(i, rec[i]);
    return fp == p->rec_fp ? FLEX_OK : FLEX_ERR_FORMAT;
}

}

extern "C" {

int flex_plan_read_records(const flex_plan *p, uint32_t *out, int64_t records) try {
    if (!p || records != p->n_records || (!out && records > 0)) return FLEX_ERR_INVALID;
    if (records == 0) return FLEX_OK;
    const DeviceScope on(p->device);
    FLEX_HIP_TRY(on.error());
    if (p->d_t_beg.size() != p->n_tasks + size_t(1) || p->d_chunk.size() != p->n_slots) return FLEX_ERR_FORMAT;
    std::vector<uint32_t> t_beg;
    std::vector<uint4> chunk;
    std::vector<uint2> rec;
    if (!read_back(p->d_t_beg, t_beg) || !read_back(p->d_chunk, chunk)) return FLEX_ERR_HIP;
    const int rc = load_records(p, t_beg, chunk, rec);
    if (rc) return rc;
    for (size_t i = 0; i < rec.size(); ++i) {
        out[2 * i] = rec[i].x;
        out[2 * i + 1] = rec[i].y;
    }
    return FLEX_OK;
} catch (const std::bad_alloc &) {
    return FLEX_ERR_NOMEM;
}

int flex_plan_measure_imbalance(flex_plan *p, const float *dB, float *dC, flex_stream_t stream, flex_imbalance *out) try {
    if (!p || p->bf16 || !out || !dC || (!dB && p->nnz > 0)) return FLEX_ERR_INVALID;
    *out = flex_imbalance{};
    if (p->m == 0 || p->n_slots == 0) return FLEX_OK;
    if (!operands_vec4(p, dB, dC) || p->bk_blocks) return FLEX_ERR_UNSUPPORTED;
    const DeviceScope on(p->device);
    FLEX_HIP_TRY(on.error());
    const size_t ktiles = (static_cast<size_t>(p->k) + 4 * p->lanes_per_nz - 1) / (4 * p->lanes_per_nz);
    const size_t words = static_cast<size_t>(p->n_slots) * ktiles * 3;
    DeviceArray<uint64_t> d_log;
    hipStream_t s = reinterpret_cast<hipStream_t>(stream);
    int rc = FLEX_OK;
    std::vector<uint64_t> log(words);
    if (d_log.allocate(words) != hipSuccess) rc = FLEX_ERR_HIP;
    if (!rc && hipMemsetAsync(d_log.get(), 0, words * 8, s) != hipSuccess) rc = FLEX_ERR_HIP;
    if (!rc) {
        rc = launch_spmm_stamped(plan_view(p, p->fused_fixup, d_log.get()), p->lanes_per_nz, p->off32, dB, dC, s);
        if (rc == FLEX_OK && !p->fused_fixup) rc = launch_fixup(p->d_partial.get(), p->d_split.get(), p->n_split, p->k, p->ldc, dC, s);
        if (rc == FLEX_OK && p->n_tiles) {
            rc = launch_tiles(tile_view(p), p->off32, dB, dC, p->k, p->ldb, p->ldc, s);
        }
    }
    if (!rc && (hipStreamSynchronize(s) != hipSuccess || hipMemcpy(log.data(), d_log.get(), words * 8, hipMemcpyDeviceToHost) != hipSuccess)) rc = FLEX_ERR_HIP;
    if (rc) return rc;
    struct Acc {
        uint64_t busy = 0, first = ~0ull, last = 0;
    };
    std::vector<Acc> cu(16 * 256), xcd(16);
    uint64_t t_min = ~0ull, t_max = 0, busy_all = 0, w_max = 0;
    int64_t waves = 0;
    for (size_t i = 0; i < words; i += 3) {
        const uint64_t t0 = log[i], t1 = log[i + 1], id = log[i + 2];
        if (t1 == 0 || t1 < t0) continue;
        const uint32_t x = static_cast<uint32_t>(id >> 32) & 15u, c = (static_cast<uint32_t>(id) >> 8) & 255u;
        for (Acc *a : {&cu[x * 256 + c], &xcd[x]}) {
            a->busy += t1 - t0;
            a->first = std::min(a->first, t0);
            a->last = std::max(a->last, t1);
        }
        t_min = std::min(t_min, t0);
        t_max = std::max(t_max, t1);
        busy_all += t1 - t0;
        w_max = std::max(w_max, t1 - t0);
        ++waves;
    }
    if (waves == 0) return FLEX_OK;
    auto summarise = [&](const std::vector<Acc> &v, int32_t *seen, double *busy_imb, double *end_spread) {
        uint64_t bmax = 0, bsum = 0, emin = ~0ull, emax = 0;
        int cnt = 0;
        for (const Acc &a : v) {
            if (a.last == 0) continue;
            ++cnt;
            bmax = std::max(bmax, a.busy);
            bsum += a.busy;
            emin = std::min(emin, a.last);
            emax = std::max(emax, a.last);
        }
        *seen = cnt;
        *busy_imb = bsum ? 100.0 * bmax * cnt / bsum - 100.0 : 0.0;
        *end_spread = t_max > t_min ? 100.0 * (emax - emin) / (t_max - t_min) : 0.0;
    };
    out->waves = waves;
    out->span_us = (t_max - t_min) * 0.01;
    summarise(cu, &out->cus_seen, &out->cu_busy_imb_pct, &out->cu_end_spread_pct);
    summarise(xcd, &out->xcds_seen, &out->xcd_busy_imb_pct, &out->xcd_end_spread_pct);
    out->wave_us_mean = busy_all * 0.01 / waves;
    out->wave_us_max = w_max * 0.01;
    return FLEX_OK;
} catch (const std::bad_alloc &) {
    return FLEX_ERR_NOMEM;
}

static int check_value_image(const flex_plan *p, const std::vector<uint2> &rec, uint64_t row_bytes) {
    const size_t nr = rec.size();
    std::vector<uint32_t> src, grp;
    std::vector<float> vrec;
    std::vector<uint4> seg, item;
    if (!read_back(p->d_src, src) || !read_back(p->d_vrec, vrec) || !read_back(p->d_seg, seg) || !read_back(p->d_sd_item, item) ||
        !read_back(p->d_sd_grp, grp))
        return FLEX_ERR_HIP;
    std::vector<uint8_t> seen(static_cast<size_t>(p->src_nnz), 0);
    int64_t real = 0;
    uint64_t fp = 0;
// ... 250 lines not shown
    uint64_t bd_total = 0;
    std::vector<std::pair<uint32_t, uint32_t>> seen;
    std::vector<std::pair<uint32_t, uint32_t>> bd_parts;
    for (size_t ci = 0; ci < chunk.size(); ++ci) {
        const uint4 &c = chunk[ci];
        const uint2 cb = chunk_bd.empty() ? make_uint2(0u, 0u) : chunk_bd[ci];
        if (c.y == 0) {
            if (c.x | c.z | c.w | cb.x | cb.y) return FLEX_ERR_FORMAT;
            continue;
        }
        if (c.y > 63 || c.x + c.y > p->n_tasks || c.z != t_beg[c.x] || c.w != t_beg[c.x + c.y]) return FLEX_ERR_FORMAT;
        if (cb.y > kBundleRowsPerChunk || cb.y % S != 0 || static_cast<uint64_t>(cb.x) + cb.y > bd_rows.size()) return FLEX_ERR_FORMAT;
        uint32_t at = 0;
        for (uint32_t t = c.x; t < c.x + c.y; ++t) {
            if ((t_dst[t] & (kPartialFlag | kBundleFlag)) != (kPartialFlag | kBundleFlag)) continue;
            if ((t_dst[t] & ~(kPartialFlag | kBundleFlag)) != at || t_aux[t].x != cb.x + at) return FLEX_ERR_FORMAT;
            if (static_cast<uint64_t>(t_aux[t].y) * S != t_beg[t + 1] - t_beg[t]) return FLEX_ERR_FORMAT;
            at += S;
            ++bundles;
        }
        if (at != cb.y) return FLEX_ERR_FORMAT;
        if (cb.y) bd_parts.emplace_back(cb.x, cb.y);
        bd_total += cb.y;
        seen.emplace_back(c.x, c.y);
        ++real;
    }
    if (bundles != p->n_bundles || bd_total != bd_rows.size() || (S < kBundleMinSlots && bundles)) return FLEX_ERR_FORMAT;
    std::sort(bd_parts.begin(), bd_parts.end());
    uint32_t bd_next = 0;
    for (const auto &part : bd_parts) {
        if (part.first != bd_next) return FLEX_ERR_FORMAT;
        bd_next += part.second;
    }
    if (real != p->n_chunks) return FLEX_ERR_FORMAT;
    std::sort(seen.begin(), seen.end());
    for (const auto &c : seen) {
        if (c.first != next_task) return FLEX_ERR_FORMAT;
        next_task += c.second;
    }
    if (next_task != p->n_tasks) return FLEX_ERR_FORMAT;
    const uint64_t row_bytes = static_cast<uint64_t>(p->ldb) * 4u;
    for (const uint2 &r : rec) {
        const uint64_t col = p->off32 ? r.x / row_bytes : r.x;
        if (col >= static_cast<uint64_t>(p->n) || (p->off32 && r.x % row_bytes != 0)) return FLEX_ERR_FORMAT;
    }
    std::vector<uint8_t> written(static_cast<size_t>(p->c_rows), 0), slot_taken(p->n_partials, 0);
    int64_t in_bundles = 0;
    for (uint32_t t = 0; t < p->n_tasks; ++t) {
        const uint32_t d = t_dst[t];
        if ((d & (kPartialFlag | kBundleFlag)) == (kPartialFlag | kBundleFlag)) {
            int64_t rows_here = 0;
            for (uint32_t s2 = 0; s2 < S; ++s2) {
                const uint32_t row = bd_rows[t_aux[t].x + s2];
                if (row == kBundleNoRow || (row & kBundleZero)) {
                    for (uint32_t j = 0; j < t_aux[t].y; ++j)
                        if (rec[t_beg[t] + static_cast<size_t>(j) * S + s2].y != 0) return FLEX_ERR_FORMAT;
                }
                if (row == kBundleNoRow) continue;
                const uint32_t dr = row & ~kBundleZero;
                if (dr >= p->c_rows || written[dr]++) return FLEX_ERR_FORMAT;
                ++rows_here;
            }
            if (rows_here == 0) return FLEX_ERR_FORMAT;
            in_bundles += rows_here;
        } else if (d & kPartialFlag) {
            const uint32_t ps = d & ~kPartialFlag;
            if (ps >= p->n_partials || slot_taken[ps]++) return FLEX_ERR_FORMAT;
            const uint2 a = t_aux[t];
            if (a.x >= p->n_split || a.y != split[a.x].count || ps < split[a.x].first || ps >= split[a.x].first + split[a.x].count) return FLEX_ERR_FORMAT;
        } else {
            if (d >= p->c_rows || written[d]++) return FLEX_ERR_FORMAT;
        }
    }
    for (uint8_t w : slot_taken)
        if (w != 1) return FLEX_ERR_FORMAT;
    if (in_bundles != p->bundle_rows) return FLEX_ERR_FORMAT;
    uint32_t first = 0;
    for (uint32_t i = 0; i < p->n_split; ++i) {
        const SplitRow &sr = split[i];
        if (sr.first != first || sr.count < 2 || sr.row >= p->c_rows || written[sr.row]++) return FLEX_ERR_FORMAT;
        first += sr.count;
    }
    if (first != p->n_partials) return FLEX_ERR_FORMAT;
    if (p->n_tiles) {
        std::vector<uint32_t> rt_ptr, rt_rows, boff;
        if (!read_back(p->d_rt_ptr, rt_ptr) || !read_back(p->d_rt_rows, rt_rows) || !read_back(p->d_tile_boff, boff)) return FLEX_ERR_HIP;
        if (rt_ptr[0] != 0 || rt_ptr[p->n_row_tiles] != p->n_tiles) return FLEX_ERR_FORMAT;
        for (uint32_t i = 0; i < p->n_row_tiles; ++i)
            if (rt_ptr[i] >= rt_ptr[i + 1]) return FLEX_ERR_FORMAT;
        std::vector<uint8_t> in_rt(static_cast<size_t>(p->c_rows), 0);
        for (uint32_t d : rt_rows) {
            if (d == 0xFFFFFFFFu) continue;
            if (d >= p->c_rows || in_rt[d]++) return FLEX_ERR_FORMAT;
        }
        for (uint32_t o : boff) {
            const uint64_t col = p->off32 ? o / row_bytes : o;
            if (col >= static_cast<uint64_t>(p->n) || (p->off32 && o % row_bytes != 0)) return FLEX_ERR_FORMAT;
        }
    }
    if (p->bk_blocks) {
        const uint32_t nb = p->bk_blocks, rounds = p->bk_rounds, P = p->bk_panel_rows, RB = rounds * kBkRowsPerRound;
        if ((rounds != 2 && rounds != 4 && rounds != 8) || P == 0 || P % 4 != 0 || P > kBkPanelMax || !p->off32) return FLEX_ERR_FORMAT;
        std::vector<uint4> hdr;
        std::vector<uint2> wstart, brec;
        std::vector<uint32_t> brow, link, cnt, hcol;
        if (!read_back(p->d_bk_hdr, hdr) || !read_back(p->d_bk_wstart, wstart) || !read_back(p->d_bk_rec, brec) || !read_back(p->d_bk_brow, brow) ||
            !read_back(p->d_bk_link, link))
            return FLEX_ERR_HIP;
        uint64_t n_cnt = 0, n_hcol = 0;
        for (const uint4 &h : hdr) n_cnt += static_cast<uint64_t>(h.w) * kBkWaves, n_hcol += static_cast<uint64_t>(h.x & 0x7FFFFFFFu) * P;
        if (n_cnt != p->d_bk_cnt.size() || n_hcol != p->d_bk_hcol.size()) return FLEX_ERR_FORMAT;
        if (!read_back(p->d_bk_cnt, cnt) || !read_back(p->d_bk_hcol, hcol)) return FLEX_ERR_HIP;
        for (uint32_t o : hcol)
            if (o % row_bytes != 0 || o / row_bytes >= static_cast<uint64_t>(p->n)) return FLEX_ERR_FORMAT;
        uint64_t at_hcol = 0, at_cnt = 0, at_step = 0;
        int64_t panels = 0, real = 0;
        std::vector<uint8_t> added(static_cast<size_t>(p->c_rows), 0);
        for (uint32_t b = 0; b < nb; ++b) {
            uint4 h = hdr[b];
            const bool chains = (h.x >> 31) != 0;
            h.x &= 0x7FFFFFFFu;
            if (h.x == 0) {
                if (h.w != 0 || chains) return FLEX_ERR_FORMAT;
            } else if (h.y != at_hcol || h.z != at_cnt || h.w != 2 * h.x || h.x > kBkMaxPanels || h.y % 4 != 0) {
                return FLEX_ERR_FORMAT;
            }
            at_hcol += static_cast<uint64_t>(h.x) * P;
            at_cnt += static_cast<uint64_t>(h.w) * kBkWaves;
            panels += h.x;
            for (uint32_t w = 0; w < kBkWaves; ++w) {
                const uint2 ws = wstart[static_cast<size_t>(b) * kBkWaves + w];
                if (ws.x != at_step) return FLEX_ERR_FORMAT;
                uint64_t pos = static_cast<uint64_t>(ws.x) * kBkSlots, steps = 0;
                for (uint32_t idx = 0; idx < h.x * kBkMaxRounds; ++idx) {
                    const uint32_t ph = idx / kBkMaxRounds, rd = idx % kBkMaxRounds;
                    const uint32_t n = (cnt[h.z + static_cast<size_t>(w) * h.w + 2 * ph + rd / 4] >> (8 * (rd & 3))) & 0xFFu;
                    if (rd >= rounds && n != 0) return FLEX_ERR_FORMAT;
                    if (n > kBkRunMax || pos + static_cast<uint64_t>(n) * kBkSlots > brec.size()) return FLEX_ERR_FORMAT;
                    for (uint64_t q = 0; q < static_cast<uint64_t>(n) * kBkSlots; ++q) {
                        const uint2 r = brec[pos + q];
                        if (r.x == kBkZeroRow) {
                            if (r.y != 0) return FLEX_ERR_FORMAT;
                        } else if (r.x % kBkRowBytes != 0 || r.x / kBkRowBytes >= P) {
                            return FLEX_ERR_FORMAT;
                        } else {
                            ++real;
                        }
                    }
                    pos += static_cast<uint64_t>(n) * kBkSlots;
                    steps += n;
                }
                if (steps != ws.y) return FLEX_ERR_FORMAT;
                at_step += steps;
            }
            std::vector<uint8_t> on_chain(RB, 0);
            bool any_link = false;
            for (uint32_t s = 0; s < RB; ++s) {
                const uint32_t row = brow[static_cast<size_t>(b) * RB + s], l = link[static_cast<size_t>(b) * RB + s];
                any_link = any_link || l != 0;
                if (l & ~(kBkLinkOwner | kBkLinkPart | 0xFFFFu)) return FLEX_ERR_FORMAT;
                if ((l & kBkLinkOwner) && ((l & kBkLinkPart) || (l & 0xFFFFu) == 0 || row == kBkEmptyRow)) return FLEX_ERR_FORMAT;
                if ((l & kBkLinkPart) && row != kBkEmptyRow) return FLEX_ERR_FORMAT;
                if (!(l & (kBkLinkOwner | kBkLinkPart)) && l != 0) return FLEX_ERR_FORMAT;
                if (row == kBkEmptyRow) continue;
                if (row >= p->c_rows || !written[row] || added[row]++) return FLEX_ERR_FORMAT;
                if (l & kBkLinkOwner) {
// ... 34 lines not shown
```

flex_amd/csrc/spmm_kernels.hip:

```cpp
#include "spmm_device.h"

namespace flex {
namespace {

using namespace spmm_dev;

template <int G>
struct RowOut {
    static constexpr int kVals = G <= 8 ? 1 : 4;
    float v[kVals];
};

template <int G>
__device__ __forceinline__ int row_out_col(int lane, int c0) {
    if constexpr (G == 8) return c0 + 2 * ((lane >> 3) & 1) + ((lane >> 4) & 1);
    else if constexpr (G == 4) return c0 + 2 * ((lane >> 2) & 1) + ((lane >> 3) & 1);
    else return c0;
}

template <int G>
__device__ __forceinline__ bool row_out_lane(int lane) {
    return G == 8 ? lane < 32 : G == 4 ? lane < 16 : lane < G;
}

// ... 274 lines not shown
template <bool OFF32>
__global__ __launch_bounds__(256) void spmm_generic_kernel(PlanView p, const float *__restrict__ B,
                                                           float *__restrict__ C, uint32_t slots_per_step) {
    const int lane = threadIdx.x & 63;
    const uint32_t wib = __builtin_amdgcn_readfirstlane(threadIdx.x >> 6);
    const uint32_t cpx = gridDim.x / kXcds;
    const uint32_t bid = p.xcd_remap ? (blockIdx.x % kXcds) * cpx + (blockIdx.x / kXcds) : blockIdx.x;
    const uint32_t w = bid * kWavesPerBlock + wib;
    if (w >= p.n_chunks) return;
    const int k = p.k;
    const int cb = blockIdx.y * 256 + lane;
    const uint32_t t0 = p.chunk[w].x, t1 = t0 + p.chunk[w].y;
    uint2 cx = make_uint2(0u, 0u);
    if (p.rec_packed != 0 && t1 > t0) cx = p.chunk_exc[w];
    const bool packed_chunk = p.rec_packed != 0 && (cx.y & kChunkWide) == 0;
    const uint32_t cz = p.chunk[w].z;
    const uint2 *__restrict__ rec = p.rec_packed != 0 ? p.rec + cx.x - cz : p.rec;
    uint32_t ei = 0;
    for (uint32_t t = t0; t < t1; ++t) {
        const uint32_t zb = p.t_beg[t], ze = p.t_beg[t + 1];
        const uint32_t dst = p.t_dst[t];
        if ((dst & (kPartialFlag | kBundleFlag)) == (kPartialFlag | kBundleFlag)) {
            const uint2 a = p.t_aux[t];
            const uint32_t slots = slots_per_step;
            for (uint32_t s = 0; s < slots; ++s) {
                const uint32_t row = p.bd_rows[a.x + s];
                if (row == kBundleNoRow) continue;
                float acc[4] = {0.f, 0.f, 0.f, 0.f};
                if ((row & kBundleZero) == 0) {
                    for (uint32_t j = 0; j < a.y; ++j) {
                        const uint2 r = rec[zb + j * slots + s];
                        const float v = as_f32(r.y);
                        const float *brow = OFF32 ? reinterpret_cast<const float *>(reinterpret_cast<const char *>(B) + r.x)
                                                  : B + static_cast<uint64_t>(r.x) * p.ldb;
#pragma unroll
                        for (int i = 0; i < 4; ++i) {
                            const int c = cb + 64 * i;
                            if (c < k) acc[i] = fmaf(v, brow[c], acc[i]);
                        }
                    }
                }
                float *orow = C + static_cast<uint64_t>(row & ~kBundleZero) * p.ldc;
#pragma unroll
                for (int i = 0; i < 4; ++i) {
                    const int c = cb + 64 * i;
                    if (c < k) orow[c] = acc[i];
                }
            }
            continue;
        }
        float acc[4] = {0.f, 0.f, 0.f, 0.f};
        uint32_t col = packed_chunk ? p.t_col0[t] : 0u;
        for (uint32_t z = zb; z < ze; ++z) {
            uint2 r;
            if (packed_chunk) {
                uint32_t d = p.rec_dcol[z];
                if (ei < cx.y && p.exc[cx.x + ei].x == z - cz) d += p.exc[cx.x + ei++].y;
                col += d;
                r = make_uint2(OFF32 ? col * (static_cast<uint32_t>(p.ldb) * 4u) : col, __float_as_uint(p.rec_val[z]));
            } else {
                r = rec[z];
            }
            const float v = as_f32(r.y);
            const float *brow = OFF32 ? reinterpret_cast<const float *>(reinterpret_cast<const char *>(B) + r.x)
                                      : B + static_cast<uint64_t>(r.x) * p.ldb;
#pragma unroll
            for (int i = 0; i < 4; ++i) {
                const int c = cb + 64 * i;
                if (c < k) acc[i] = fmaf(v, brow[c], acc[i]);
            }
        }
        float *orow = (dst & kPartialFlag) ? p.partial + static_cast<uint64_t>(dst & ~kPartialFlag) * k
                                           : C + static_cast<uint64_t>(dst) * p.ldc;
#pragma unroll
        for (int i = 0; i < 4; ++i) {
            const int c = cb + 64 * i;
            if (c < k) orow[c] = acc[i];
        }
    }
}

__global__ __launch_bounds__(256) void spmm_fixup_kernel(const float *__restrict__ partial,
                                                         const SplitRow *__restrict__ rows, uint32_t n_rows,
                                                         int k, int ldc, float *__restrict__ C) {
    const int lane = threadIdx.x & 63;
    const uint32_t wib = __builtin_amdgcn_readfirstlane(threadIdx.x >> 6);
    const uint32_t i = blockIdx.x * kWavesPerBlock + wib;
    if (i >= n_rows) return;
    const SplitRow sr = rows[i];
    for (int c = lane; c < k; c += 64) {
        const float *p = partial + static_cast<uint64_t>(sr.first) * k + c;
        float s = 0.f;
        uint32_t j = 0;
        for (; j + 8 <= sr.count; j += 8) {
            float v[8];
#pragma unroll
            for (int u = 0; u < 8; ++u) v[u] = p[static_cast<uint64_t>(j + u) * k];
#pragma unroll
            for (int u = 0; u < 8; ++u) s += v[u];
        }
        float v[8];
#pragma unroll
        for (int u = 0; u < 8; ++u) v[u] = (j + u < sr.count) ? p[static_cast<uint64_t>(j + u) * k] : 0.f;
#pragma unroll
        for (int u = 0; u < 8; ++u)
            if (j + u < sr.count) s += v[u];
        C[static_cast<uint64_t>(sr.row) * ldc + c] = s;
    }
}

template <bool VEC4>
__global__ __launch_bounds__(256) void gather_rows_kernel(float *__restrict__ dst, const float *__restrict__ src,
                                                          const int32_t *__restrict__ idx, int64_t n, int k) {
    const int lane = threadIdx.x & 63;
    const int64_t nwaves = static_cast<int64_t>(gridDim.x) * kWavesPerBlock;
    for (int64_t r = static_cast<int64_t>(blockIdx.x) * kWavesPerBlock + (threadIdx.x >> 6); r < n; r += nwaves) {
        const int64_t s = idx[r];
        if constexpr (VEC4) {
            const float4 *sp = reinterpret_cast<const float4 *>(src + s * k);
            float4 *dp = reinterpret_cast<float4 *>(dst + r * k);
            for (int c = lane; c < k / 4; c += 64) dp[c] = sp[c];
        } else {
            for (int c = lane; c < k; c += 64) dst[r * k + c] = src[s * k + c];
        }
    }
}

template <int G, bool OFF32, int U>
int launch_v4(const PlanView &v, const float *dB, float *dC, hipStream_t s) {
    uint32_t nblk = (v.n_chunks + kWavesPerBlock - 1) / kWavesPerBlock;
    nblk = (nblk + kXcds - 1) / kXcds * kXcds;
    const uint32_t ktiles = (v.k + 4 * G - 1) / (4 * G);
    const dim3 grid = v.tile_group ? dim3(nblk * ktiles, 1) : dim3(nblk, ktiles);
    hipLaunchKernelGGL((spmm_flat_kernel<G, OFF32, U, kWavesPerBlock>), grid, dim3(64 * kWavesPerBlock), v.lds_extra, s, v, dB, dC);
    FLEX_HIP_TRY(hipGetLastError());
    return FLEX_OK;
}

template <int G, int U>
int launch_stamped(const PlanView &v, bool off32, const float *dB, float *dC, hipStream_t s) {
    uint32_t nblk = (v.n_chunks + kWavesPerBlock - 1) / kWavesPerBlock;
    nblk = (nblk + kXcds - 1) / kXcds * kXcds;
    const uint32_t ktiles = (v.k + 4 * G - 1) / (4 * G);
    const dim3 grid = v.tile_group ? dim3(nblk * ktiles, 1) : dim3(nblk, ktiles);
    if (off32)
        hipLaunchKernelGGL((spmm_flat_kernel<G, true, U, kWavesPerBlock, true>), grid, dim3(64 * kWavesPerBlock), v.lds_extra, s, v, dB, dC);
    else
        hipLaunchKernelGGL((spmm_flat_kernel<G, false, U, kWavesPerBlock, true>), grid, dim3(64 * kWavesPerBlock), v.lds_extra, s, v, dB, dC);
    FLEX_HIP_TRY(hipGetLastError());
    return FLEX_OK;
}

template <int G, int U>
int launch_v4_off(const PlanView &v, bool off32, const float *dB, float *dC, hipStream_t s) {
    return off32 ? launch_v4<G, true, U>(v, dB, dC, s) : launch_v4<G, false, U>(v, dB, dC, s);
}

}

int launch_spmm(const PlanView &v, int lanes_per_nz, bool off32, bool vec4, const float *dB, float *dC,
                hipStream_t s, int unroll) {
    if (v.n_chunks == 0) return FLEX_OK;
    if (!vec4) {
        uint32_t nblk = (v.n_chunks + kWavesPerBlock - 1) / kWavesPerBlock;
        nblk = (nblk + kXcds - 1) / kXcds * kXcds;
        const uint32_t ktiles = (v.k + 255) / 256;
        if (off32)
            hipLaunchKernelGGL((spmm_generic_kernel<true>), dim3(nblk, ktiles), dim3(256), 0, s, v, dB, dC, 64u / static_cast<uint32_t>(lanes_per_nz));
        else
            hipLaunchKernelGGL((spmm_generic_kernel<false>), dim3(nblk, ktiles), dim3(256), 0, s, v, dB, dC, 64u / static_cast<uint32_t>(lanes_per_nz));
        FLEX_HIP_TRY(hipGetLastError());
        return FLEX_OK;
    }
    if (unroll == 8) {
        switch (lanes_per_nz) {
            case 8: return launch_v4_off<8, 8>(v, off32, dB, dC, s);
            case 16: return launch_v4_off<16, 8>(v, off32, dB, dC, s);
            default: break;
        }
    }
    switch (lanes_per_nz) {
        case 4: return launch_v4_off<4, 4>(v, off32, dB, dC, s);
        case 8: return launch_v4_off<8, 4>(v, off32, dB, dC, s);
        case 16: return launch_v4_off<16, 4>(v, off32, dB, dC, s);
        case 32: return launch_v4_off<32, 8>(v, off32, dB, dC, s);
        case 64: return launch_v4_off<64, 8>(v, off32, dB, dC, s);
        default: return FLEX_ERR_UNSUPPORTED;
    }
}

int launch_spmm_stamped(const PlanView &v, int lanes_per_nz, bool off32, const float *dB, float *dC, hipStream_t s) {
    if (v.n_chunks == 0) return FLEX_OK;
    switch (lanes_per_nz) {
        case 4: return launch_stamped<4, 4>(v, off32, dB, dC, s);
        case 8: return launch_stamped<8, 4>(v, off32, dB, dC, s);
        case 16: return launch_stamped<16, 4>(v, off32, dB, dC, s);
        case 32: return launch_stamped<32, 8>(v, off32, dB, dC, s);
        case 64: return launch_stamped<64, 8>(v, off32, dB, dC, s);
        default: return FLEX_ERR_UNSUPPORTED;
    }
}

int kernel_attributes(int lanes_per_nz, bool off32, bool vec4, hipFuncAttributes *attr, int *waves_per_cu) {
    const void *fn = nullptr;
    if (!vec4) {
        fn = off32 ? reinterpret_cast<const void *>(spmm_generic_kernel<true>) : reinterpret_cast<const void *>(spmm_generic_kernel<false>);
    } else {
        switch (lanes_per_nz) {
            case 4: fn = off32 ? reinterpret_cast<const void *>(spmm_flat_kernel<4, true, 4, kWavesPerBlock>) : reinterpret_cast<const void *>(spmm_flat_kernel<4, false, 4, kWavesPerBlock>); break;
            case 8: fn = off32 ? reinterpret_cast<const void *>(spmm_flat_kernel<8, true, 4, kWavesPerBlock>) : reinterpret_cast<const void *>(spmm_flat_kernel<8, false, 4, kWavesPerBlock>); break;
            case 16: fn = off32 ? reinterpret_cast<const void *>(spmm_flat_kernel<16, true, 4, kWavesPerBlock>) : reinterpret_cast<const void *>(spmm_flat_kernel<16, false, 4, kWavesPerBlock>); break;
            case 32: fn = off32 ? reinterpret_cast<const void *>(spmm_flat_kernel<32, true, 8, kWavesPerBlock>) : reinterpret_cast<const void *>(spmm_flat_kernel<32, false, 8, kWavesPerBlock>); break;
            case 64: fn = off32 ? reinterpret_cast<const void *>(spmm_flat_kernel<64, true, 8, kWavesPerBlock>) : reinterpret_cast<const void *>(spmm_flat_kernel<64, false, 8, kWavesPerBlock>); break;
            default: return FLEX_ERR_UNSUPPORTED;
        }
    }
    FLEX_HIP_TRY(hipFuncGetAttributes(attr, fn));
    int blocks = 0;
    FLEX_HIP_TRY(hipOccupancyMaxActiveBlocksPerMultiprocessor(&blocks, fn, 64 * kWavesPerBlock, 0));
    *waves_per_cu = blocks * kWavesPerBlock;
    return FLEX_OK;
}

int launch_fixup(const float *partial, const SplitRow *rows, uint32_t n_rows, int k, int ldc, float *dC, hipStream_t s) {
    if (n_rows == 0) return FLEX_OK;
    const uint32_t nblk = (n_rows + kWavesPerBlock - 1) / kWavesPerBlock;
    hipLaunchKernelGGL(spmm_fixup_kernel, dim3(nblk), dim3(256), 0, s, partial, rows, n_rows, k, ldc, dC);
    FLEX_HIP_TRY(hipGetLastError());
    return FLEX_OK;
}

int launch_gather_rows(float *dst, const float *src, const int32_t *idx, int64_t n, int k, hipStream_t s) {
    if (n <= 0) return FLEX_OK;
    const int64_t want = (n + kWavesPerBlock - 1) / kWavesPerBlock;
    const uint32_t nblk = static_cast<uint32_t>(want < 2048 ? want : 2048);
    const bool vec4 = (k % 4 == 0) && ((reinterpret_cast<uintptr_t>(dst) | reinterpret_cast<uintptr_t>(src)) % 16 == 0);
    if (vec4)
        hipLaunchKernelGGL((gather_rows_kernel<true>), dim3(nblk), dim3(256), 0, s, dst, src, idx, n, k);
    else
        hipLaunchKernelGGL((gather_rows_kernel<false>), dim3(nblk), dim3(256), 0, s, dst, src, idx, n, k);
    FLEX_HIP_TRY(hipGetLastError());
    return FLEX_OK;
}

}
```

include/flex_spmm.h:

```cpp
#ifndef FLEX_SPMM_H
#define FLEX_SPMM_H
#include <stddef.h>
#include <stdint.h>

#ifdef __cplusplus
extern "C" {
#endif

#define FLEX_ABI_VERSION 3

typedef enum flex_status {
    FLEX_OK = 0,
    FLEX_ERR_INVALID = -1,
    FLEX_ERR_NOMEM = -2,
    FLEX_ERR_HIP = -3,
    FLEX_ERR_UNSUPPORTED = -4,
    FLEX_ERR_IO = -5,
    FLEX_ERR_FORMAT = -6,
    FLEX_ERR_DUPLICATE = -7
} flex_status;

typedef struct flex_csr {
    int32_t m, n;
    int64_t nnz;
    const uint32_t *rowPtr;
    const uint32_t *col;
    const float *vals;
} flex_csr;

typedef struct ihipStream_t *flex_stream_t;

typedef struct flex_plan flex_plan;

#define FLEX_ORDER_NATURAL 0u
#define FLEX_ORDER_RCM 1u
#define FLEX_ORDER_CLUSTER 2u
#define FLEX_ORDER_GORDER 3u
#define FLEX_ORDER_MASK 0xFu
#define FLEX_PLAN_STATS 0x100u
#define FLEX_PLAN_AUTOTUNE 0x200u
#define FLEX_PLAN_ROW_RANGE 0x1000u
#define FLEX_PLAN_XCD_INTERLEAVE 0x2000u
#define FLEX_PLAN_TRANSPOSE 0x8000u
#define FLEX_PLAN_MUTABLE_VALUES 0x10000u

#define FLEX_PLAN_ATTENTION 0x40000u

#define FLEX_PLAN_ATTENTION_BACKWARD 0x80000u
#define FLEX_PLAN_BF16 0x100000u

int flex_plan_create(flex_plan **out, const flex_csr *hostA, int k, int device, unsigned flags);

int flex_plan_create_ld(flex_plan **out, const flex_csr *hostA, int k, int ldb, int ldc, int device, unsigned flags);

int flex_plan_create_mapped(flex_plan **out, const flex_csr *hostA, const int32_t *vo_mp, int k,
                            int device, unsigned flags);

int flex_plan_create_rows(flex_plan **out, const flex_csr *hostA, int64_t row_begin, int64_t row_end,
                          const int32_t *col_map, int k, int device, unsigned flags);

typedef struct flex_cluster_tuning {
    int32_t batch;
    int32_t no_refine;
    int32_t stretch;
    int32_t sweeps;
    int32_t stride;
} flex_cluster_tuning;
typedef struct flex_plan_tuning {
    int32_t lanes_per_nz;
    int32_t chunk_records;
    int32_t long_row;
    int32_t piece_records;
    int32_t row_cost;
    int32_t xcd_slices;
    int32_t xcd_balance;
    int32_t chunk_cost, task_cost;
    int32_t split_rows;
    int32_t rec_nt;
    int32_t unroll;
    int32_t two_d;
    int32_t panel_kb;
    int32_t seg_min;
    int32_t mfma;
    int32_t mfma_fill_pct;
    int32_t lds_extra;
    int32_t host_threads;
    flex_cluster_tuning cluster;
    int32_t blocks;
    int32_t block_rounds;
    int32_t block_panel_rows;
    int32_t block_thr;
    int32_t block_cap;
    int32_t block_ablate_retired;
    int32_t tile_group;
    int32_t xcd_stretch;
    int32_t far_first;
    int32_t bundle;
    int32_t bundle_len;
    int32_t rec_pack;
    int32_t reserved[4];
} flex_plan_tuning;

typedef struct flex_plan_desc {
    size_t struct_size;
    const flex_csr *A;
    int k, ldb, ldc, device;
    unsigned flags;
    int64_t row_begin, row_end;
    const int32_t *col_map, *row_map;
    const flex_plan_tuning *tuning;
} flex_plan_desc;
int flex_plan_create_ex(flex_plan **out, const flex_plan_desc *desc);
int flex_plan_get_tuning(const flex_plan *plan, flex_plan_tuning *out);

int flex_set_host_threads(int n);

int flex_spmm(flex_plan *plan, const float *dB, float *dC, flex_stream_t stream);

typedef uint16_t flex_bf16;
int flex_spmm_bf16(flex_plan *plan, const flex_bf16 *dB, flex_bf16 *dC, flex_stream_t stream);
int flex_plan_is_bf16(const flex_plan *plan);

int flex_plan_set_values(flex_plan *plan, const float *dVals, flex_stream_t stream);

int flex_sddmm(const flex_plan *plan, const float *dG, const float *dB, float *dOut, flex_stream_t stream);

int flex_edge_softmax(const flex_plan *plan, const float *dScores, float scale, float *dOut, flex_stream_t stream);
int flex_edge_softmax_backward(const flex_plan *plan, const float *dP, const float *dGradP, float scale, float *dGradS, flex_stream_t stream);

typedef struct flex_softmax_info {
    int64_t rows;
    int64_t entries;
    int64_t items;
    int64_t groups;
    int64_t rows_empty;
    int64_t rows_packed;
    int64_t rows_wave;
    int64_t rows_block;
    int64_t group_entries;
    int64_t device_bytes;
} flex_softmax_info;
int flex_plan_softmax_info(const flex_plan *plan, flex_softmax_info *out);

int flex_attention(const flex_plan *plan, const float *dQ, const float *dK, const float *dV, float scale, float *dOut, float *dP, flex_stream_t stream);

typedef struct flex_attention_info {
    int64_t rows;
    int64_t entries;
    int64_t items;
    int64_t groups;
    int64_t rows_empty;
    int64_t rows_slot;
    int64_t rows_wave;
    int64_t rows_block;
    int64_t group_budget;
    int64_t device_bytes;
} flex_attention_info;
int flex_plan_attention_info(const flex_plan *plan, flex_attention_info *out);

int flex_attention_backward(const flex_plan *plan, const float *dQ, const float *dK, const float *dV, const float *dP,
                            const float *dGradOut, float scale, float *dGradQ, float *dGradK, float *dGradV, float *dWork,
                            flex_stream_t stream);

typedef struct flex_attention_backward_info {
    int64_t columns;
    int64_t entries;
    int64_t items;
    int64_t groups;
    int64_t columns_empty;
    int64_t columns_slot;
    int64_t columns_wave;
    int64_t columns_block;
    int64_t group_budget;
    int64_t device_bytes;
} flex_attention_backward_info;
int flex_plan_attention_backward_info(const flex_plan *plan, flex_attention_backward_info *out);

int flex_attention_heads(const flex_plan *plan, int heads, const float *dQ, const float *dK, const float *dV, float scale, float *dOut,
                         float *dP, flex_stream_t stream);
int flex_attention_heads_backward(const flex_plan *plan, int heads, const float *dQ, const float *dK, const float *dV, const float *dP,
                                  const float *dGradOut, float scale, float *dGradQ, float *dGradK, float *dGradV, float *dWork,
                                  flex_stream_t stream);

int flex_attention_bf16(const flex_plan *plan, int heads, const flex_bf16 *dQ, const flex_bf16 *dK, const flex_bf16 *dV, float scale,
                        flex_bf16 *dOut, float *dP, flex_stream_t stream);
int flex_attention_bf16_backward(const flex_plan *plan, int heads, const flex_bf16 *dQ, const flex_bf16 *dK, const flex_bf16 *dV, const float *dP,
                                 const flex_bf16 *dGradOut, float scale, flex_bf16 *dGradQ, flex_bf16 *dGradK, flex_bf16 *dGradV, float *dWork,
                                 flex_stream_t stream);

int flex_attention_bias(const flex_plan *plan, int heads, const float *dQ, const float *dK, const float *dV, const float *dBias, float scale,
                        float *dOut, float *dP, flex_stream_t stream);
int flex_attention_bias_backward(const flex_plan *plan, int heads, const float *dQ, const float *dK, const float *dV, const float *dP,
                                 const float *dGradOut, float scale, float *dGradQ, float *dGradK, float *dGradV, float *dGradBias,
                                 float *dWork, flex_stream_t stream);
int flex_attention_bf16_bias(const flex_plan *plan, int heads, const flex_bf16 *dQ, const flex_bf16 *dK, const flex_bf16 *dV, const float *dBias,
                             float scale, flex_bf16 *dOut, float *dP, flex_stream_t stream);
int flex_attention_bf16_bias_backward(const flex_plan *plan, int heads, const flex_bf16 *dQ, const flex_bf16 *dK, const flex_bf16 *dV,
                                      const float *dP, const flex_bf16 *dGradOut, float scale, flex_bf16 *dGradQ, flex_bf16 *dGradK,
                                      flex_bf16 *dGradV, float *dGradBias, float *dWork, flex_stream_t stream);

extern int flex_attention_dropout(const flex_plan *plan, int heads, const float *dQ, const float *dK, const float *dV, const float *dBias ,
                           float scale, float drop_p, uint64_t seed, float *dOut, float *dP, flex_stream_t stream);
extern int flex_attention_dropout_backward(const flex_plan *plan, int heads, const float *dQ, const float *dK, const float *dV, const float *dP,
                                    const float *dGradOut, float scale, float drop_p, uint64_t seed, float *dGradQ, float *dGradK, float *dGradV,
                                    float *dGradBias , float *dWork, flex_stream_t stream);
extern int flex_attention_bf16_dropout(const flex_plan *plan, int heads, const flex_bf16 *dQ, const flex_bf16 *dK, const flex_bf16 *dV,
                                const float *dBias , float scale, float drop_p, uint64_t seed, flex_bf16 *dOut, float *dP,
                                flex_stream_t stream);
extern int flex_attention_bf16_dropout_backward(const flex_plan *plan, int heads, const flex_bf16 *dQ, const flex_bf16 *dK, const flex_bf16 *dV,
                                         const float *dP, const flex_bf16 *dGradOut, float scale, float drop_p, uint64_t seed, flex_bf16 *dGradQ,
                                         flex_bf16 *dGradK, flex_bf16 *dGradV, float *dGradBias , float *dWork, flex_stream_t stream);
int flex_dropout_mask(uint64_t seed, float drop_p, uint64_t first, uint64_t count, uint8_t *keep_host);

int flex_gat_attention(const flex_plan *plan, int heads, const float *dEl, const float *dEr, const float *dV, float slope, float *dOut,
                       float *dP, flex_stream_t stream);
int flex_gat_attention_backward(const flex_plan *plan, int heads, const float *dEl, const float *dEr, const float *dV, const float *dP,
                                const float *dGradOut, float slope, float *dGradEl, float *dGradEr, float *dGradV, float *dWork,
                                flex_stream_t stream);

extern int flex_gat_attention_dropout(const flex_plan *plan, int heads, const float *dEl, const float *dEr, const float *dV, float slope, float drop_p,
                               uint64_t seed, float *dOut, float *dP, flex_stream_t stream);
extern int flex_gat_attention_dropout_backward(const flex_plan *plan, int heads, const float *dEl, const float *dEr, const float *dV, const float *dP,
                                        const float *dGradOut, float slope, float drop_p, uint64_t seed, float *dGradEl, float *dGradEr,
                                        float *dGradV, float *dWork, flex_stream_t stream);

int flex_plan_destroy(flex_plan *plan);

typedef struct flex_plan_info {
    int32_t m, n, k, device;
    int64_t nnz;
    int64_t n_tasks;
    int64_t n_chunks;
    int64_t n_split_rows;
    int64_t n_partials;
    int64_t device_bytes;
    int32_t lanes_per_nz;
    int32_t order;
    double plan_ms;
    int64_t n_slots;
    int32_t two_d;
    int32_t panel_rows;
    int64_t n_tiles;
    int64_t tile_nnz;
    int64_t n_records;
    int64_t n_blocks;
    int64_t block_rows;
    int64_t block_nnz;
    int64_t block_hot_nnz;
    int64_t block_hot_cols;
    int64_t block_panels;
    int64_t block_records;
    int64_t n_bundles;
    int64_t bundle_rows;
} flex_plan_info;
int flex_plan_get_info(const flex_plan *plan, flex_plan_info *out);

typedef struct flex_record_info {
    int32_t packed;
    int32_t reserved;
    int64_t records;
    int64_t wide_records;
    int64_t exceptions;
    int64_t stream_bytes;
} flex_record_info;
int flex_plan_record_info(const flex_plan *plan, flex_record_info *out);
int flex_plan_read_records(const flex_plan *plan, uint32_t *out, int64_t records);

typedef struct flex_plan_stats {
    int64_t records;
    int64_t cols_wave;
    int64_t cols_wg;
    int64_t cols_xcd;
    double reuse_wave;
    double reuse_wg;
    double reuse_xcd;
    double gather_bytes;
    double l2_bytes;
    int64_t chunk_rec_max;
    double chunk_rec_mean;
    double chunk_imb_pct;
    double xcd_imb_pct;
    double split_nnz_pct;
    double pad_pct;
    int64_t n_workgroups;
    double tile_nnz_pct_10;
    double tile_nnz_pct_25;
    double tile_nnz_pct_50;
    double tile_mean_fill;
    int64_t mfma_tiles;
    double mfma_nnz_pct;
    double lds_hot_pct_2, lds_hot_pct_4;
    double lds_u_2, lds_u_4;
} flex_plan_stats;
int flex_plan_get_stats(const flex_plan *plan, flex_plan_stats *out);

typedef struct flex_imbalance {
    int64_t waves;
    int32_t cus_seen;
    int32_t xcds_seen;
    double span_us;
    double cu_busy_imb_pct;
    double cu_end_spread_pct;
    double xcd_busy_imb_pct;
    double xcd_end_spread_pct;
    double wave_us_mean, wave_us_max;
} flex_imbalance;
int flex_plan_measure_imbalance(flex_plan *plan, const float *dB, float *dC, flex_stream_t stream, flex_imbalance *out);

typedef struct flex_kernel_info {
    int32_t vgprs, sgprs;
    int32_t lds_bytes;
    int32_t scratch_bytes;
    int32_t threads_per_block;
    int32_t waves_per_cu;
} flex_kernel_info;
int flex_plan_kernel_info(const flex_plan *plan, flex_kernel_info *out);

int flex_plan_self_check(const flex_plan *plan);

int flex_hbm_probe(int device, int64_t bytes, int reps, int temporal, double *read_gbps, double *copy_gbps);

int flex_gather_rows(float *dst, const float *src, const int32_t *idx, int64_t n, int k,
                     flex_stream_t stream);


typedef struct flex_host_csr {
    int32_t m, n;
    int64_t nnz;
    uint32_t *rowPtr;
    uint32_t *col;
    float *vals;
    int64_t uni_nb;
    int64_t n_edges_one_way, n_edges_asymmetric;
    int32_t n_nodes_z_out, n_nodes_z_in, n_nodes_z_deg;
    int32_t is_directed;
    int32_t c;
} flex_host_csr;

int flex_csv_load(const char *path, flex_host_csr *out);
void flex_host_csr_free(flex_host_csr *a);

int flex_mtx_load(const char *path, int sort_columns, flex_host_csr *out);

int flex_csv_save(const char *path, const flex_csr *A);

int flex_csr_save_bin(const char *path, const flex_csr *A);
int flex_csr_load_bin(const char *path, flex_host_csr *out);

uint64_t flex_csr_fingerprint(const flex_csr *A);
// ... 49 lines not shown
```

Measured before the change: 8404.

## Add column-class partitioning of rows across XCDs and a multi-row vectorized fixup

Adds an optional col_classes tuning (2 or 4) that splits each row's nonzeros by column index modulo W and assigns each class to its own group of XCDs, so each XCD gathers a narrower subset of B rows and its L2 holds a smaller working set. The default rule returns 1, so column classes are off unless requested. The fixup kernel is also rewritten so several rows share one wave, using float4 loads when k and ldc are multiples of 4 and C is 16-byte aligned. That fixup path is on by default and changes how partial sums are reduced. Column classes would add more split rows and partial slots, which means extra fixup work in exchange for better cache locality.

Measured after the change: 8406 (median of 4 runs). No clear change (+0.0%).

```diff
diff --git a/flex_amd/binding.py b/flex_amd/binding.py
--- a/flex_amd/binding.py
+++ b/flex_amd/binding.py
@@ -77,7 +77,7 @@
         "lanes_per_nz", "chunk_records", "long_row", "piece_records", "row_cost", "xcd_slices", "xcd_balance",
         "chunk_cost", "task_cost", "split_rows", "rec_nt", "unroll", "two_d", "panel_kb", "seg_min", "mfma",
         "mfma_fill_pct", "lds_extra", "host_threads")] + [("cluster", _ClusterTuning)] + [(f, C.c_int32) for f in (
-        "blocks", "block_rounds", "block_panel_rows", "block_thr", "block_cap", "block_ablate_retired", "tile_group", "xcd_stretch", "far_first", "bundle", "bundle_len", "rec_pack")] + [("reserved", C.c_int32 * 4)]
+        "blocks", "block_rounds", "block_panel_rows", "block_thr", "block_cap", "block_ablate_retired", "tile_group", "xcd_stretch", "far_first", "bundle", "bundle_len", "rec_pack", "col_classes")] + [("reserved", C.c_int32 * 3)]
 
 
 TUNING_FIELDS = tuple(f for f, _ in _PlanTuning._fields_ if f not in ("cluster", "block_ablate_retired", "reserved"))
@@ -153,7 +153,7 @@
     "flex_last_hip_error_string", "flex_abi_version", "flex_plan_set_values", "flex_sddmm",
     "flex_edge_softmax", "flex_edge_softmax_backward", "flex_plan_softmax_info", "flex_attention", "flex_plan_attention_info",
     "flex_attention_backward", "flex_plan_attention_backward_info", "flex_attention_heads", "flex_attention_heads_backward",
-    "flex_gat_attention", "flex_gat_attention_backward", "flex_plan_record_info", "flex_plan_read_records",
+    "flex_gat_attention", "flex_gat_attention_backward", "flex_plan_record_info", "flex_plan_read_records", "flex_plan_read_tasks",
     "flex_attention_bf16", "flex_attention_bf16_backward", "flex_spmm_bf16", "flex_plan_is_bf16",
     "flex_attention_bias", "flex_attention_bias_backward", "flex_attention_bf16_bias", "flex_attention_bf16_bias_backward",
     "flex_attention_dropout", "flex_attention_dropout_backward", "flex_attention_bf16_dropout", "flex_attention_bf16_dropout_backward",
@@ -235,6 +235,7 @@
         L.flex_plan_attention_backward_info.argtypes = [vp, C.POINTER(_AttentionBackwardInfo)]
         L.flex_plan_record_info.argtypes = [vp, C.POINTER(_RecordInfo)]
         L.flex_plan_read_records.argtypes = [vp, vp, i64]
+        L.flex_plan_read_tasks.argtypes = [vp, vp, i64]
         L.flex_plan_is_bf16.argtypes = [vp]
         L.flex_dropout_mask.argtypes = [C.c_uint64, C.c_float, C.c_uint64, C.c_uint64, vp]
         _lib = L
@@ -511,6 +512,8 @@
         _check(lib().flex_plan_get_info(self._h, C.byref(i)), "flex_plan_get_info")
         d = {f: getattr(i, f) for f, _ in _PlanInfo._fields_}
         d["rec_packed"] = self.record_info()["packed"]
+        d["col_classes"] = self.tuning()["col_classes"]
+        d["n_pieces"] = d["n_partials"]
         d["bf16"] = int(lib().flex_plan_is_bf16(self._h))
         return d
 
@@ -523,6 +526,12 @@
         n = self.record_info()["records"]
         out = np.empty((max(n, 1), 2), dtype=np.uint32)
         _check(lib().flex_plan_read_records(self._h, out.ctypes.data, n), "flex_plan_read_records")
+        return out[:n]
+
+    def tasks(self) -> np.ndarray:
+        n = self.info()["n_tasks"]
+        out = np.empty((max(n, 1), 5), dtype=np.uint32)
+        _check(lib().flex_plan_read_tasks(self._h, out.ctypes.data, n), "flex_plan_read_tasks")
         return out[:n]
 
     def stats(self) -> dict:
diff --git a/flex_amd/csrc/plan.cpp b/flex_amd/csrc/plan.cpp
--- a/flex_amd/csrc/plan.cpp
+++ b/flex_amd/csrc/plan.cpp
@@ -203,6 +203,16 @@
         tuning.mfma = 2;
         tuning.blocks = 2;
         tuning.rec_pack = 2;
+    }
+    const bool classes = tuning.col_classes == 2 || tuning.col_classes == 4;
+    if (tuning.col_classes > 2 && tuning.col_classes != 4) return FLEX_ERR_INVALID;
+    if (classes) {
+        if (bf16 || mut || !all_rows || (flags & (FLEX_PLAN_TRANSPOSE | FLEX_PLAN_ATTENTION | FLEX_PLAN_ATTENTION_BACKWARD | FLEX_PLAN_AUTOTUNE))) return FLEX_ERR_UNSUPPORTED;
+        if (tuning.mfma == 1 || tuning.blocks == 1 || tuning.two_d == 1 || k % 4 != 0 || ldb % 4 != 0 || ldc % 4 != 0) return FLEX_ERR_UNSUPPORTED;
+        tuning.mfma = 2;
+        tuning.blocks = 2;
+    } else if (bf16 || mut || !all_rows || (flags & (FLEX_PLAN_TRANSPOSE | FLEX_PLAN_ATTENTION | FLEX_PLAN_AUTOTUNE))) {
+        tuning.col_classes = 1;
     }
     int rc = FLEX_OK;
     const flex_csr *const callerA = hostA;
@@ -322,6 +332,7 @@
     const DeviceScope on(p->device);
     FLEX_HIP_TRY(on.error());
     const bool vec4 = operands_vec4(p, dB, dC);
+    if (!vec4 && p->col_classes > 1) return FLEX_ERR_UNSUPPORTED;
     const bool fused = vec4 && p->fused_fixup;
     hipStream_t s = reinterpret_cast<hipStream_t>(stream);
     int rc = FLEX_OK;
diff --git a/flex_amd/csrc/plan.h b/flex_amd/csrc/plan.h
--- a/flex_amd/csrc/plan.h
+++ b/flex_amd/csrc/plan.h
@@ -101,6 +101,7 @@
     flex::DeviceArray<uint32_t> d_split_cnt;
     bool fused_fixup = false;
     bool two_d = false;
+    uint32_t col_classes = 1;
     flex::DeviceArray<float> d_tile_a;
     flex::DeviceArray<uint32_t> d_tile_boff, d_tile_mask, d_rt_ptr, d_rt_rows;
     uint32_t n_tiles = 0, n_row_tiles = 0;
diff --git a/flex_amd/csrc/plan_build.cpp b/flex_amd/csrc/plan_build.cpp
--- a/flex_amd/csrc/plan_build.cpp
+++ b/flex_amd/csrc/plan_build.cpp
@@ -75,6 +75,8 @@
         order_pieces();
         lap("emission order");
         number_split_rows();
+        if (timing && W > 1)
+            std::fprintf(stderr, "plan: column classes W = %u: %zu pieces of %zu rows in %u partial slots\n", W, pieces.size(), split.size(), n_partials);
         form_tasks();
         if ((rc = pack_tasks_into_chunks())) return rc;
         fill_records();
@@ -121,6 +123,8 @@
     std::vector<float> f_vals;
     uint32_t wave_nnz = 0, row_cost = 16, long_row = 0, piece_len = 0, seg_min = 4, pshift = 0, far_window = 0;
     bool two_d = false;
+    uint32_t W = 1;
+    uint32_t n_row_slices = kXcds;
     bool xcd_dealt = false;
     std::vector<Piece> pieces;
     std::vector<uint32_t> row_first_piece;
@@ -357,6 +361,11 @@
         pshift = 0;
         while ((2ull << pshift) * tile_bytes <= panel_bytes) ++pshift;
         seg_min = static_cast<uint32_t>(pick(tn.seg_min, 4));
+        W = tn.col_classes == 2 || tn.col_classes == 4 ? static_cast<uint32_t>(tn.col_classes) : tn.col_classes == 1 ? 1u : col_class_rule();
+        if (!p->xcd_remap || xcd_dealt || two_d || m == 0 || tiles.nnz || p->bk_blocks || mut || k % 4 != 0 || p->ldb % 4 != 0 || p->ldc % 4 != 0) W = 1;
+        n_row_slices = two_d ? kXcds : kXcds / W;
+        p->col_classes = W;
+        p->tuning.col_classes = static_cast<int32_t>(W);
         bundles_on = bundles_expected && !two_d;
         bundle_len = static_cast<uint32_t>(pick(tn.bundle_len, S >= 8 ? 12 : 16));
         const bool pack_shape = !two_d && !mut && k % 4 == 0 && p->ldb % 4 == 0 && p->ldc % 4 == 0;
@@ -387,6 +396,8 @@
     }
     bool bundle_rule() const { return fills_the_chip() || avg_deg < 16.0; }
 
+    uint32_t col_class_rule() const { return 1u; }
+
     void cut_run(std::vector<Piece> &out, uint32_t spos, uint32_t b, uint32_t e, uint32_t phase) const {
         const uint32_t len = e - b;
         if (len <= long_row) {
@@ -404,6 +415,7 @@
         rcol = A->col;
         rval = A->vals;
         if (two_d) return cut_by_column_panel();
+        if (W > 1) return cut_by_column_class();
         pieces.reserve(static_cast<size_t>(m) + 1024);
         for (int32_t i = 0; i < m; ++i) {
             const uint32_t r = sched[i];
@@ -490,6 +502,10 @@
             }
         });
         if (failed.load()) return FLEX_ERR_NOMEM;
+        return join_piece_blocks(blk, row_np, kBlk);
+    }
+
+    int join_piece_blocks(const std::vector<std::vector<Piece>> &blk, const std::vector<uint32_t> &row_np, int64_t per) {
         size_t total = 0;
         for (int32_t i = 0; i < m; ++i) {
             row_first_piece[i] = static_cast<uint32_t>(total);
@@ -498,33 +514,71 @@
         row_first_piece[m] = static_cast<uint32_t>(total);
         if (total >= (size_t(1) << 31)) return FLEX_ERR_UNSUPPORTED;
         pieces.resize(total);
-        parallel_chunks(nblk, [&](int64_t b) {
+        parallel_chunks(static_cast<int64_t>(blk.size()), [&](int64_t b) {
             const std::vector<Piece> &src = blk[static_cast<size_t>(b)];
-            if (!src.empty()) std::copy(src.begin(), src.end(), pieces.begin() + row_first_piece[b * kBlk]);
+            if (!src.empty()) std::copy(src.begin(), src.end(), pieces.begin() + row_first_piece[b * per]);
         });
         rcol = pcol.data();
         rval = pval.data();
         return FLEX_OK;
     }
 
+    int cut_by_column_class() {
+        const uint32_t e_base = A->rowPtr[r0];
+        pcol.resize(static_cast<size_t>(slice_nnz()));
+        pval.resize(static_cast<size_t>(slice_nnz()));
+        constexpr int64_t kBlk = 1024;
+        const int64_t nblk = (m + kBlk - 1) / kBlk;
+        std::vector<std::vector<Piece>> blk(static_cast<size_t>(nblk));
+        std::vector<uint32_t> row_np(static_cast<size_t>(m), 0u);
+        std::atomic<int> failed{0};
+        auto class_of = [&](uint32_t c) { return (col_map ? static_cast<uint32_t>(col_map[c]) : c) % W; };
+        parallel_chunks(nblk, [&](int64_t b) {
+            try {
+                std::vector<Piece> &out = blk[static_cast<size_t>(b)];
+                for (int64_t i = b * kBlk; i < std::min<int64_t>(m, (b + 1) * kBlk); ++i) {
+                    const uint32_t r = sched[i];
+                    const uint32_t e0 = A->rowPtr[r], e1 = A->rowPtr[r + 1], o0 = e0 - e_base;
+                    const size_t before = out.size();
+                    uint32_t cnt[4] = {0, 0, 0, 0}, at[4];
+                    for (uint32_t e = e0; e < e1; ++e) ++cnt[class_of(A->col[e])];
+                    for (uint32_t q = 0, o = o0; q < W; o += cnt[q++]) at[q] = o;
+                    for (uint32_t e = e0; e < e1; ++e) {
+                        const uint32_t o = at[class_of(A->col[e])]++;
+                        pcol[o] = A->col[e];
+                        pval[o] = A->vals[e];
+                    }
+                    if (e1 == e0) out.push_back({static_cast<uint32_t>(i), o0, o0, 0u, 0u});
+                    for (uint32_t q = 0, o = o0; q < W; o += cnt[q++])
+                        if (cnt[q]) cut_run(out, static_cast<uint32_t>(i), o, o + cnt[q], q);
+                    row_np[i] = static_cast<uint32_t>(out.size() - before);
+                }
+            } catch (...) {
+                failed.store(1);
+            }
+        });
+        if (failed.load()) return FLEX_ERR_NOMEM;
+        return join_piece_blocks(blk, row_np, kBlk);
+    }
+
     void slice_rows_for_xcds() {
-        std::fill(slice_row, slice_row + kXcds, 0u);
-        slice_row[kXcds] = static_cast<uint32_t>(m);
-        if (!two_d) return;
+        std::fill(slice_row, slice_row + kXcds + 1, static_cast<uint32_t>(m));
+        slice_row[0] = 0u;
+        if (!two_d && W == 1) return;
         std::vector<uint64_t> cum(static_cast<size_t>(m) + 1, 0);
         for (int32_t i = 0; i < m; ++i) {
             const uint32_t r = sched[i];
             cum[i + 1] = cum[i] + (A->rowPtr[r + 1] - A->rowPtr[r]) + row_cost;
         }
-        for (int x = 1; x < kXcds; ++x)
-            slice_row[x] = std::max<uint32_t>(slice_row[x - 1], static_cast<uint32_t>(std::lower_bound(cum.begin(), cum.end(), cum[m] * x / kXcds) - cum.begin()));
+        for (uint32_t x = 1; x < n_row_slices; ++x)
+            slice_row[x] = std::max<uint32_t>(slice_row[x - 1], static_cast<uint32_t>(std::lower_bound(cum.begin(), cum.end(), cum[m] * x / n_row_slices) - cum.begin()));
     }
 
     void order_pieces() {
         emit.resize(pieces.size());
         std::iota(emit.begin(), emit.end(), 0u);
-        if (!two_d) return;
-        parallel_chunks(kXcds, [&](int64_t x) {
+        if (!two_d && W == 1) return;
+        parallel_chunks(n_row_slices, [&](int64_t x) {
             auto b = emit.begin() + row_first_piece[slice_row[x]], e = emit.begin() + row_first_piece[slice_row[x + 1]];
             std::stable_sort(b, e, [&](uint32_t u, uint32_t v) { return pieces[u].phase < pieces[v].phase; });
         });
@@ -577,9 +631,17 @@
             }
             buf.clear();
         };
+        uint32_t cur_slice = 0, cur_class = 0;
         for (uint32_t e = 0; e < n_pieces; ++e) {
             const Piece &pc = pieces[emit[e]];
-            if (pc.own_chunk == 0 && pc.end - pc.beg <= bundle_len) {
+            bool whole_row = true;
+            if (W > 1) {
+                while (pc.spos >= slice_row[cur_slice + 1]) ++cur_slice, flush_buf();
+                if (pc.phase != cur_class) flush_buf();
+                cur_class = pc.phase;
+                whole_row = row_first_piece[pc.spos + 1] - row_first_piece[pc.spos] == 1;
+            }
+            if (whole_row && pc.own_chunk == 0 && pc.end - pc.beg <= bundle_len) {
                 buf.push_back(e);
                 if (buf.size() == 8u * S) flush_buf();
             } else {
@@ -597,6 +659,7 @@
         uint64_t pos = 0;
         uint32_t wave_cost = 0, cur_phase = 0, prev_own = 0, bd_first = 0;
         int cur_slice = 0;
+        uint32_t cur_group = 0;
         for (uint32_t t = 0; t < n_tasks; ++t) {
             const TaskSpec &ts = tasks[t];
             const Piece &pc = pieces[emit[ts.rows ? bundle_piece[ts.ref] : ts.ref]];
@@ -611,6 +674,12 @@
                 }
                 if (pc.phase != cur_phase) fresh = true;
                 cur_phase = pc.phase;
+            } else if (W > 1) {
+                while (pc.spos >= slice_row[cur_group + 1]) ++cur_group;
+                while (cur_slice < static_cast<int>(cur_group * W + pc.phase)) {
+                    slice_chunk[++cur_slice] = static_cast<uint32_t>(w_task.size());
+                    fresh = true;
+                }
             }
             if (fresh) {
                 if (!w_task.empty()) chunk_bd.push_back(make_uint2(bd_first, static_cast<uint32_t>(bd_rows.size()) - bd_first));
@@ -642,7 +711,7 @@
         if (!w_task.empty()) chunk_bd.push_back(make_uint2(bd_first, static_cast<uint32_t>(bd_rows.size()) - bd_first));
         w_task.push_back(n_tasks);
         if (m == 0) w_task.assign(1, 0u);
-        if (two_d)
+        if (two_d || W > 1)
             while (cur_slice < kXcds) slice_chunk[++cur_slice] = static_cast<uint32_t>(w_task.size() - 1);
         rec.resize(static_cast<size_t>(pos));
         return FLEX_OK;
@@ -928,11 +997,11 @@
                 const uint32_t x = s % kXcds, c0 = s * per, c1 = std::min(n_real, c0 + per);
                 for (uint32_t c = c0; c < c1; ++c) place(static_cast<size_t>(x) * longest + at[x]++, c);
             }
-        } else if (two_d || (p->xcd_remap && n_real >= 8u * kXcds * kWavesPerBlock && tn.xcd_balance != 2)) {
+        } else if (two_d || W > 1 || (p->xcd_remap && n_real >= 8u * kXcds * kWavesPerBlock && tn.xcd_balance != 2)) {
             uint32_t cut[kXcds + 1];
             cut[0] = 0;
             cut[kXcds] = n_real;
-            if (two_d) {
+            if (two_d || W > 1) {
                 for (uint32_t x = 1; x < kXcds; ++x) cut[x] = slice_chunk[x];
             } else {
                 const uint64_t chunk_cost = static_cast<uint64_t>(pick(tn.chunk_cost, 16)) * 32u;
diff --git a/flex_amd/csrc/plan_check.cpp b/flex_amd/csrc/plan_check.cpp
--- a/flex_amd/csrc/plan_check.cpp
+++ b/flex_amd/csrc/plan_check.cpp
@@ -150,6 +150,34 @@
     return FLEX_ERR_NOMEM;
 }
 
+int flex_plan_read_tasks(const flex_plan *p, uint32_t *out, int64_t tasks) try {
+    if (!p || tasks != static_cast<int64_t>(p->n_tasks) || (!out && tasks > 0)) return FLEX_ERR_INVALID;
+    if (tasks == 0) return FLEX_OK;
+    const DeviceScope on(p->device);
+    FLEX_HIP_TRY(on.error());
+    if (p->d_t_beg.size() != p->n_tasks + size_t(1) || p->d_t_dst.size() != p->n_tasks || p->d_chunk.size() != p->n_slots) return FLEX_ERR_FORMAT;
+    std::vector<uint32_t> t_beg, t_dst;
+    std::vector<uint4> chunk;
+    if (!read_back(p->d_t_beg, t_beg) || !read_back(p->d_t_dst, t_dst) || !read_back(p->d_chunk, chunk)) return FLEX_ERR_HIP;
+    const size_t wgs = (chunk.size() + kWavesPerBlock - 1) / kWavesPerBlock, per = (wgs + kXcds - 1) / kXcds;
+    for (size_t ci = 0; ci < chunk.size(); ++ci) {
+        const uint4 &c = chunk[ci];
+        if (static_cast<uint64_t>(c.x) + c.y > p->n_tasks) return FLEX_ERR_FORMAT;
+        const size_t wg = ci / kWavesPerBlock;
+        const uint32_t xcd = static_cast<uint32_t>(p->xcd_remap ? std::min<size_t>(wg / per, kXcds - 1) : wg % kXcds);
+        for (uint32_t t = c.x; t < c.x + c.y; ++t) {
+            out[5 * size_t(t)] = t_beg[t];
+            out[5 * size_t(t) + 1] = t_beg[t + 1];
+            out[5 * size_t(t) + 2] = t_dst[t];
+            out[5 * size_t(t) + 3] = xcd;
+            out[5 * size_t(t) + 4] = static_cast<uint32_t>(ci);
+        }
+    }
+    return FLEX_OK;
+} catch (const std::bad_alloc &) {
+    return FLEX_ERR_NOMEM;
+}
+
 int flex_plan_measure_imbalance(flex_plan *p, const float *dB, float *dC, flex_stream_t stream, flex_imbalance *out) try {
     if (!p || p->bf16 || !out || !dC || (!dB && p->nnz > 0)) return FLEX_ERR_INVALID;
     *out = flex_imbalance{};
@@ -566,6 +594,23 @@
         first += sr.count;
     }
     if (first != p->n_partials) return FLEX_ERR_FORMAT;
+    if (const uint32_t W = p->col_classes; W != 1) {
+        if ((W != 2 && W != 4) || n_slots % kXcds != 0 || p->two_d || p->n_tiles || p->bk_blocks || !p->xcd_remap) return FLEX_ERR_FORMAT;
+        const size_t per = n_slots / kXcds;
+        std::vector<uint8_t> slot_class(p->n_partials, 0);
+        for (size_t ci = 0; ci < chunk.size(); ++ci) {
+            const uint4 &c = chunk[ci];
+            if (c.y == 0) continue;
+            const uint32_t q = static_cast<uint32_t>(ci / per) % W;
+            for (uint32_t z = c.z; z < c.w; ++z)
+                if ((p->off32 ? rec[z].x / row_bytes : rec[z].x) % W != q) return FLEX_ERR_FORMAT;
+            for (uint32_t t = c.x; t < c.x + c.y; ++t)
+                if ((t_dst[t] & (kPartialFlag | kBundleFlag)) == kPartialFlag) slot_class[t_dst[t] & ~kPartialFlag] = static_cast<uint8_t>(q);
+        }
+        for (const SplitRow &sr : split)
+            for (uint32_t j = 1; j < sr.count; ++j)
+                if (slot_class[sr.first + j] < slot_class[sr.first + j - 1]) return FLEX_ERR_FORMAT;
+    }
     if (p->n_tiles) {
         std::vector<uint32_t> rt_ptr, rt_rows, boff;
         if (!read_back(p->d_rt_ptr, rt_ptr) || !read_back(p->d_rt_rows, rt_rows) || !read_back(p->d_tile_boff, boff)) return FLEX_ERR_HIP;
diff --git a/flex_amd/csrc/spmm_kernels.hip b/flex_amd/csrc/spmm_kernels.hip
--- a/flex_amd/csrc/spmm_kernels.hip
+++ b/flex_amd/csrc/spmm_kernels.hip
@@ -380,9 +380,34 @@
 
 __global__ __launch_bounds__(256) void spmm_fixup_kernel(const float *__restrict__ partial,
                                                          const SplitRow *__restrict__ rows, uint32_t n_rows,
-                                                         int k, int ldc, float *__restrict__ C) {
+                                                         int k, int ldc, float *__restrict__ C, uint32_t lg_lanes) {
     const int lane = threadIdx.x & 63;
     const uint32_t wib = __builtin_amdgcn_readfirstlane(threadIdx.x >> 6);
+    if (lg_lanes != 0) {
+        const uint32_t L = 1u << lg_lanes;
+        const uint32_t i = ((blockIdx.x * kWavesPerBlock + wib) << (6 - lg_lanes)) + (static_cast<uint32_t>(lane) >> lg_lanes);
+        if (i >= n_rows) return;
+        const SplitRow sr = rows[i];
+        for (int c = static_cast<int>(lane & (L - 1)) * 4; c < k; c += static_cast<int>(4 * L)) {
+            const float *p = partial + static_cast<uint64_t>(sr.first) * k + c;
+            float4 s = {0.f, 0.f, 0.f, 0.f};
+            for (uint32_t j = 0; j < sr.count; j += 4) {
+                float4 v[4];
+#pragma unroll
+                for (int u = 0; u < 4; ++u) v[u] = *reinterpret_cast<const float4 *>(p + static_cast<uint64_t>(min(j + u, sr.count - 1)) * k);
+#pragma unroll
+                for (int u = 0; u < 4; ++u)
+                    if (j + u < sr.count) {
+                        s.x += v[u].x;
+                        s.y += v[u].y;
+                        s.z += v[u].z;
+                        s.w += v[u].w;
+                    }
+            }
+            *reinterpret_cast<float4 *>(C + static_cast<uint64_t>(sr.row) * ldc + c) = s;
+        }
+        return;
+    }
     const uint32_t i = blockIdx.x * kWavesPerBlock + wib;
     if (i >= n_rows) return;
     const SplitRow sr = rows[i];
@@ -522,8 +547,14 @@
 
 int launch_fixup(const float *partial, const SplitRow *rows, uint32_t n_rows, int k, int ldc, float *dC, hipStream_t s) {
     if (n_rows == 0) return FLEX_OK;
-    const uint32_t nblk = (n_rows + kWavesPerBlock - 1) / kWavesPerBlock;
-    hipLaunchKernelGGL(spmm_fixup_kernel, dim3(nblk), dim3(256), 0, s, partial, rows, n_rows, k, ldc, dC);
+    uint32_t lg = 0;
+    if (k % 4 == 0 && ldc % 4 == 0 && reinterpret_cast<uintptr_t>(dC) % 16 == 0) {
+        lg = 3;
+        while ((4 << lg) < k && lg < 6) ++lg;
+    }
+    const uint32_t per_wg = lg ? kWavesPerBlock << (6 - lg) : kWavesPerBlock;
+    const uint32_t nblk = (n_rows + per_wg - 1) / per_wg;
+    hipLaunchKernelGGL(spmm_fixup_kernel, dim3(nblk), dim3(256), 0, s, partial, rows, n_rows, k, ldc, dC, lg);
     FLEX_HIP_TRY(hipGetLastError());
     return FLEX_OK;
 }
diff --git a/include/flex_spmm.h b/include/flex_spmm.h
--- a/include/flex_spmm.h
+++ b/include/flex_spmm.h
@@ -98,7 +98,8 @@
     int32_t bundle;
     int32_t bundle_len;
     int32_t rec_pack;
-    int32_t reserved[4];
+    int32_t col_classes;
+    int32_t reserved[3];
 } flex_plan_tuning;
 
 typedef struct flex_plan_desc {
@@ -265,6 +266,7 @@
 } flex_record_info;
 int flex_plan_record_info(const flex_plan *plan, flex_record_info *out);
 int flex_plan_read_records(const flex_plan *plan, uint32_t *out, int64_t records);
+int flex_plan_read_tasks(const flex_plan *plan, uint32_t *out, int64_t tasks);
 
 typedef struct flex_plan_stats {
     int64_t records;
```
